# hengdashi/cuda_gcn

Measured on AMD Instinct MI355X. Metric: epochs_per_sec, higher is better.
Workload: dtype f32

## Files before the change

cuda_gcn_amd/_lib.py:

```python
from __future__ import annotations

import ctypes as C
import os

HERE = os.path.dirname(os.path.abspath(__file__))
LIBDIR = os.environ.get("GCN_LIBDIR") or os.path.join(HERE, "lib")

_cache = {}


class NativeLibraryMissing(RuntimeError):
    pass


def _load(name: str) -> C.CDLL:
    if name in _cache:
        return _cache[name]
    path = os.path.join(LIBDIR, name)
    if not os.path.exists(path):
        raise NativeLibraryMissing(
            f"{path} not found: the HIP extension is not built. Run `make kernels host` "
            f"(or __graft_entry__.build()); there is no CPU fallback.")
    try:
        lib = C.CDLL(path)
    except OSError as e:
        raise NativeLibraryMissing(f"cannot load {path}: {e}") from e
    _cache[name] = lib
    return lib


def gcnhip() -> C.CDLL:
    lib = _load("libgcnhip.so")
    if not getattr(lib, "_typed", False):
        _declare_gcnhip(lib)
        lib._typed = True
    return lib


def gcnhost() -> C.CDLL:
    gcnhip()
    lib = _load("libgcnhost.so")
    if not getattr(lib, "_typed", False):
        _declare_gcnhost(lib)
        lib._typed = True
    return lib


P = C.c_void_p
I = C.c_int
I64 = C.c_int64
U64 = C.c_uint64
F = C.c_float


class AdamVar(C.Structure):
    _fields_ = [("w", P), ("g", P), ("m", P), ("v", P), ("n", I64), ("decay", I)]


GCNHIP_SYMBOLS = {
    "gcnhip_device_count": (I, [C.POINTER(I)]),
    "gcnhip_ctx_create": (I, [C.POINTER(P), I, P]),
    "gcnhip_ctx_destroy": (I, [P]),
    "gcnhip_ctx_sync": (I, [P]),
    "gcnhip_ctx_set_corun": (I, [P, I]),
    "gcnhip_ctx_set_option": (I, [P, C.c_char_p, I]),
    "gcnhip_ctx_get_option": (I, [P, C.c_char_p, C.POINTER(I)]),
    "gcnhip_ctx_stream": (P, [P]),
    "gcnhip_error_string": (C.c_char_p, [I]),
    "gcnhip_last_error": (C.c_char_p, []),
    "gcnhip_version": (C.c_char_p, []),
    "gcnhip_experiments": (I, []),
    "gcnhip_malloc": (I, [P, C.POINTER(P), C.c_size_t]),
    "gcnhip_free": (I, [P, P]),
    "gcnhip_memset_async": (I, [P, P, I, C.c_size_t]),
    "gcnhip_h2d": (I, [P, P, P, C.c_size_t]),
    "gcnhip_d2h": (I, [P, P, P, C.c_size_t]),
    "gcnhip_d2d_async": (I, [P, P, P, C.c_size_t]),
    "gcnhip_host_alloc": (I, [C.POINTER(P), C.c_size_t]),
    "gcnhip_host_free": (I, [P]),
    "gcnhip_d2h_async": (I, [P, P, P, C.c_size_t]),
    "gcnhip_graph_create": (I, [P, C.POINTER(P), P, P, I, I, P]),
    "gcnhip_graph_create_grouped": (I, [P, C.POINTER(P), P, P, I, I, P, P]),
    "gcnhip_graph_set_schedule": (I, [P, P, I, P, I]),
    "gcnhip_graph_reserve_width": (I, [P, P, I]),
    "gcnhip_graph_destroy": (I, [P, P]),
    "gcnhip_graph_arrays": (I, [P, C.POINTER(P), C.POINTER(P), C.POINTER(P), C.POINTER(I), C.POINTER(I)]),
    "gcnhip_graphsum": (I, [P, P, P, I, P, I, I]),
    "gcnhip_graphsum_rowmask": (I, [P, P, P, I, P, I, I, P]),
    "gcnhip_graphsum_masked": (I, [P, P, P, I, P, I, I, P, P]),
    "gcnhip_graph_add_rowset": (I, [P, P, P, C.POINTER(P)]),
    "gcnhip_graph_create_restricted": (I, [P, C.POINTER(P), P, P]),
    "gcnhip_graph_clone": (I, [P, C.POINTER(P), P]),
    "gcnhip_rowset_size": (I, [P, C.POINTER(I)]),
    "gcnhip_graphsum_rowset": (I, [P, P, P, P, I, P, I, I, P]),
    "gcnhip_graphsum_relu_dropout": (I, [P, P, P, I, P, I, I, I, F, U64, P, U64, P]),
    "gcnhip_graphsum_relu_dropout_bits": (I, [P, P, P, I, P, I, I, I, F, U64, P, U64, P, P, I]),
    "gcnhip_graphsum_ex": (I, [P, P, P, P, I, P, I, I]),
    "gcnhip_graphsum_predict": (I, [P, P, P, P, P, I, P, I, I, I, P, P, P, I]),
    "gcnhip_graphsum_blend": (I, [P, P, P, I, P, I, P, I, I, F, F, F, F, P]),
    "gcnhip_cs_error_rows": (I, [P, P, I, P, I, P, I, I, P, I, P]),
    "gcnhip_cs_correct_rows": (I, [P, P, I, P, I, P, I, I, P, P, I]),
    "gcnhip_calib_nll_rows": (I, [P, P, I, P, I, P, I, I, F, P]),
    "gcnhip_calib_bins_rows": (I, [P, P, I, P, I, P, I, I, F, I, P, P, P]),
    "gcnhip_calib_scale_rows": (I, [P, P, I, I, P, I, I, F, P, I, P]),
    "gcnhip_embed_inv_norms": (I, [P, P, I, I, I, P]),
    "gcnhip_topk_plan": (I, [I, I, I, I, C.POINTER(I), C.POINTER(I), C.POINTER(C.c_size_t), C.POINTER(C.c_size_t)]),
    "gcnhip_topk_rows": (I, [P, P, I, I, I, P, P, P, I, I, I, I, P, C.c_size_t, I, P, P]),
    "gcnhip_pair_scores": (I, [P, P, I, I, I, P, P, P, I, P]),
    "gcnhip_embed_rows": (I, [P, P, I, I, I, P, P, I, P, I]),
    "gcnhip_graph_remove_rowset": (I, [P, P, P]),
    "gcnhip_graph_scales": (I, [P, C.POINTER(P), C.POINTER(P), C.POINTER(P), C.POINTER(P)]),
    "gcnhip_feat_scale_rows": (I, [P, P, P]),
    "gcnhip_xent_fwd_rows_scaled": (I, [P, P, I, P, I, P, P, I, I, I, I, I, P, P, P]),
    "gcnhip_xent_from_row_terms": (I, [P, P, P, P, I, P, P]),
    "gcnhip_matmul_bwd_ex": (I, [P, P, I, P, I, P, I, P, I, P, I, I, I, I, F, P, I, P]),
    "gcnhip_graphsum_part": (I, [P, P, P, P, I, P, I, I, P, I, I, I, F, U64, P, U64, P]),
    "gcnhip_feat_create": (I, [P, C.POINTER(P), P, P, P, I, I]),
    "gcnhip_feat_create_aggregated": (I, [P, C.POINTER(P), P, P]),
    "gcnhip_feat_destroy": (I, [P, P]),
    "gcnhip_feat_is_dense": (I, [P]),
    "gcnhip_feat_values": (P, [P]),
    "gcnhip_feat_nnz": (I64, [P]),
    "gcnhip_spmm_fwd": (I, [P, P, P, P, I, P, I, I, F, U64, P, U64, P]),
    "gcnhip_spmm_fwd_relu": (I, [P, P, P, P, I, P, I, I]),
    "gcnhip_spmm_fwd_relu_matmul": (I, [P, P, P, P, I, I, P, I, I, P, I]),
    "gcnhip_spmm_bwd": (I, [P, P, P, P, I, P, I, I, F, U64, P, U64, P]),
    "gcnhip_spmm_bwd_plan": (I, [P, P, I, C.POINTER(I), C.POINTER(I)]),
    "gcnhip_spmm_bwd_part": (I, [P, P, P, P, I, I, F, U64, P, U64, P, I, I, I]),
    "gcnhip_spmm_bwd_finish": (I, [P, P, P, I, I]),
    "gcnhip_matmul_fwd": (I, [P, P, I, P, I, P, I, I, I, I]),
    "gcnhip_matmul_bwd": (I, [P, P, I, P, I, P, I, P, I, P, I, I, I, I]),
    "gcnhip_matmul_bwd_fused": (I, [P, P, I, P, I, P, I, P, I, P, I, I, I, I, F]),
    "gcnhip_matmul_bwd_fused_bits": (I, [P, P, I, P, I, P, I, P, I, P, I, I, I, I, F, P, I]),
    "gcnhip_pack_positive": (I, [P, P, I, I, I, P, I]),
    "gcnhip_f32_to_bf16": (I, [P, P, I, P, I, I64, I]),
    "gcnhip_graphsum_bf16": (I, [P, P, P, I, P, I, I, P, P, I, I, F, U64, P, U64, P]),
    "gcnhip_matmul_bwd_da_bits": (I, [P, P, I, P, I, P, I, I, I, I, P, I, F]),
    "gcnhip_gather_rows": (I, [P, P, I, P, I, P]),
    "gcnhip_relu_fwd": (I, [P, P, P, I64, I]),
    "gcnhip_relu_bwd": (I, [P, P, P, I64]),
    "gcnhip_dropout_fwd": (I, [P, P, P, I64, F, U64, P, U64, P]),
    "gcnhip_dropout_bwd": (I, [P, P, P, I64, F]),
    "gcnhip_relu_fwd_2d": (I, [P, P, I, I, I, P, I]),
    "gcnhip_relu_bwd_2d": (I, [P, P, I, I, I, P]),
    "gcnhip_dropout_fwd_2d": (I, [P, P, I, I, I, P, F, U64, P, U64, P]),
    "gcnhip_dropout_bwd_2d": (I, [P, P, I, I, I, P, F]),
    "gcnhip_relu_dropout_bwd": (I, [P, P, I, P, I, I, I, F]),
    "gcnhip_xent_fwd": (I, [P, P, I, P, I, P, I, I, I, I, I, P, P]),
    "gcnhip_xent_fwd_rows": (I, [P, P, I, P, I, P, P, I, I, I, I, I, P, P]),
    "gcnhip_accuracy": (I, [P, P, I, P, I, I, P]),
    "gcnhip_set_truth": (I, [P, P, P, P, I, I]),
    "gcnhip_sumsq": (I, [P, P, I64, P]),
    "gcnhip_adam_step": (I, [P, C.POINTER(AdamVar), I, F, P, P, F, F, F, F, P]),
    "gcnhip_adam_step_advance": (I, [P, C.POINTER(AdamVar), I, F, P, P, F, F, F, F, P, P, P]),
    "gcnhip_counter_add": (I, [P, P, C.c_uint32]),
    "gcnhip_metrics_record": (I, [P, P, I, I, P, P, P, P]),
    "gcnhip_metrics_record_with_next_loss": (I, [P, P, I, I, P, P]),
    "gcnhip_capture_begin": (I, [P]),
    "gcnhip_capture_end": (I, [P, C.POINTER(P)]),
    "gcnhip_graph_launch": (I, [P, P]),
    "gcnhip_graph_exec_destroy": (I, [P]),
    "gcnhip_event_create": (I, [C.POINTER(P)]),
    "gcnhip_event_create_sync": (I, [C.POINTER(P)]),
    "gcnhip_event_destroy": (I, [P]),
    "gcnhip_event_record": (I, [P, P]),
    "gcnhip_stream_wait_event": (I, [P, P]),
    "gcnhip_event_elapsed_ms": (I, [P, P, C.POINTER(F)]),
    "gcnhip_event_sync": (I, [P]),
    "gcnhip_bce_fwd_rows": (I, [P, P, I, P, I, P, I, P, I, I, I, I, P, P, P]),
    "gcnhip_bce_predict_rows": (I, [P, P, I, P, I, I, P, I, P, I]),
    "gcnhip_confusion_rows": (I, [P, P, P, I, P, I, I, P, P]),
    "gcnhip_bce_class_counts_rows": (I, [P, P, I, P, I, P, I, I, P]),
    "gcnhip_wxent_fwd_rows": (I, [P, P, I, P, I, P, P, I, I, I, I, I, P, P, P, P, F]),
    "gcnhip_wbce_fwd_rows": (I, [P, P, I, P, I, P, I, P, I, I, I, I, P, P, P, P]),
}


def _declare_gcnhip(lib):
    for name, (res, args) in GCNHIP_SYMBOLS.items():
        fn = getattr(lib, name)
# ... 93 lines not shown
```

cuda_gcn_amd/csrc/dense_bf16x3.h:

```cpp
#pragma once
#include "dense_persist.h"
#include "bf16x3_split.h"

constexpr int BX_BK = 32;
constexpr int BX_BH_BYTES = 3 * 4 * 1024;
constexpr int BX_NB = 10;
constexpr int BX_PD = 6;
constexpr int BX_SMEM = BX_NB * BX_BH_BYTES;


__device__ inline void bx_pack_w_body(int idx, const float *__restrict__ w, int ldw, int K, int n_hs, uint4 *__restrict__ wp, float scale) {
    if (idx >= n_hs * 4 * 64) return;
    const int lane = idx & 63, n = (idx >> 6) & 3, hs = idx >> 8;
    const int col = 32 * n + (lane & 31), k0 = 32 * (hs >> 1) + 16 * (lane >> 5) + 8 * (hs & 1);
    BxPlanes P;
#pragma unroll
    for (int i = 0; i < 4; i++) {
        const int k = k0 + 2 * i;
        const float a = k < K ? w[(size_t)k * ldw + col] * scale : 0.f, b = (k + 1) < K ? w[(size_t)(k + 1) * ldw + col] * scale : 0.f;
        bx_split2(a, b, P.w[0][i], P.w[1][i], P.w[2][i]);
    }
#pragma unroll
    for (int p = 0; p < 3; p++) wp[(((size_t)hs * 3 + p) * 4 + n) * 64 + lane] = make_uint4(P.w[p][0], P.w[p][1], P.w[p][2], P.w[p][3]);
}
// ... 81 lines not shown
__global__ __launch_bounds__(256) void dropbits_bx_pack_w_kernel(BxBitsArgs b, int n_bits_wgs,
                                                                 const float *__restrict__ w, int ldw, int K, int n_hs,
                                                                 uint4 *__restrict__ wp, float scale) {
    __shared__ uint32_t lds[BX_BITS_LDS_WORDS];
    if ((int)blockIdx.x < n_bits_wgs) dropbits_cm_body(blockIdx.x, threadIdx.x, b, lds);
    else bx_pack_w_body(((int)blockIdx.x - n_bits_wgs) * 256 + threadIdx.x, w, ldw, K, n_hs, wp, scale);
}

struct Bx3FwdArgs {
    const float *x; int ldx;
    const uint4 *wp;
    float *out; int ldo;
    int m, K, n_chunks, n_rb;
    const uint32_t *bits;
    int relu;
    const uint4 *w2p;
    float *z0; int ldz, p2;
};
constexpr int BX_W2_BYTES = 8 * 2 * 3 * 1024;

struct BxB3 { bf16x8 h, m, l; };
template <int N> struct BxN { static constexpr int value = N; };
struct BxRaw { f32x4 v[4]; uint32_t kw; };

template <int OFF>
__device__ __forceinline__ void bx_gload16(f32x4 &dst, const float *p) {
    asm volatile("global_load_dwordx4 %0, %1, off offset:%2" : "=v"(dst) : "v"(p), "n"(OFF) : "memory");
}
__device__ __forceinline__ void bx_gload4(uint32_t &dst, const uint32_t *p) {
    asm volatile("global_load_dword %0, %1, off" : "=v"(dst) : "v"(p) : "memory");
}
template <int OFF>
__device__ __forceinline__ void bx_ldsread16(bf16x8 &dst, uint32_t addr) {
    asm volatile("ds_read_b128 %0, %1 offset:%2" : "=v"(dst) : "v"(addr), "n"(OFF) : "memory");
}
#define BX_WAIT_LDS(b) asm volatile("s_waitcnt lgkmcnt(0)" : "+v"((b).h), "+v"((b).m), "+v"((b).l) :: "memory")
#define BX_PIN(P, i) asm volatile("" : "+v"((P).w[0][i]), "+v"((P).w[1][i]), "+v"((P).w[2][i]))
#define BX_WAIT_RAW(N, r) asm volatile("s_waitcnt vmcnt(" #N ")" : "+v"((r).v[0]), "+v"((r).v[1]), "+v"((r).v[2]), "+v"((r).v[3]), "+v"((r).kw) :: "memory")

template <bool DROP, int NP, bool ZOUT = false>
__global__ __launch_bounds__(512, 2) void dense_fwd_bf16x3_kernel(Bx3FwdArgs a) {
    constexpr int NBV = ZOUT ? 8 : BX_NB;
    static_assert(NBV >= BX_PD + 1, "ring too short for the prefetch distance");
    __shared__ __attribute__((aligned(1024))) unsigned char smem[NBV * BX_BH_BYTES + (ZOUT ? BX_W2_BYTES : 0)];
    const int tid = threadIdx.x, lane = tid & 63;
    const int wave = __builtin_amdgcn_readfirstlane(tid >> 6);
    const int li = lane & 31, hh = lane >> 5;
    const uint32_t lds0 = (uint32_t)(uintptr_t)(__attribute__((address_space(3))) unsigned char *)smem;
    if (a.m < 0) smem[tid] = 0;

    const int rb_lo = (int)((int64_t)blockIdx.x * a.n_rb / gridDim.x);
    const int nb = (int)((int64_t)(blockIdx.x + 1) * a.n_rb / gridDim.x) - rb_lo;
    if (nb <= 0) return;
    const int row_last = min(a.m, (rb_lo + nb) * 32) - 1;
    const int n_rounds = (nb + 7) / 8;
    const int n_items = n_rounds * a.n_chunks;
    const int n_hs = 2 * a.n_chunks;
    const int piece2 = wave < 4 ? wave + 8 : wave - 4;

    auto load_raw = [&](BxRaw &r, int t, int c) __attribute__((always_inline)) {
        const int row = min((rb_lo + 8 * t + wave) * 32 + li, row_last);
        const float *p = a.x + (size_t)row * a.ldx + c * BX_BK + 16 * hh;
        if (DROP) bx_gload4(r.kw, a.bits + (size_t)c * a.m + row);
        bx_gload16<0>(r.v[0], p); bx_gload16<16>(r.v[1], p); bx_gload16<32>(r.v[2], p); bx_gload16<48>(r.v[3], p);
        if (!DROP) r.kw = 0u;
    };
    auto issue_b = [&](int hq) __attribute__((always_inline)) {
        int hs = hq % n_hs;
        const uint32_t dst = lds0 + (hq % NBV) * BX_BH_BYTES;
        const uint4 *src = a.wp + (size_t)hs * (BX_BH_BYTES / 16);
        pg_glds16(src + wave * 64 + lane, dst + wave * 1024);
        pg_glds16(src + piece2 * 64 + lane, dst + piece2 * 1024);
    };
    static_assert(2 * (BX_PD - 2) == 8, "BX_WAIT_W spells the count out");
#define BX_WAIT_W() PG_WAIT_BARRIER(8)

    f32x16 acc[4];
#pragma unroll
    for (int n = 0; n < 4; n++)
#pragma unroll
        for (int r = 0; r < 16; r++) acc[n][r] = 0.f;

    const __amdgpu_buffer_rsrc_t orsrc = __builtin_amdgcn_make_buffer_rsrc(a.out, 0, (int)((uint32_t)a.m * (uint32_t)a.ldo * 4u), 0x00020000);
    auto store_block = [&](f32x16 &v, int row0, int col, bool live) __attribute__((always_inline)) {
#pragma unroll
        for (int r = 0; r < 16; r++) {
            const int row = row0 + (r & 3) + 8 * (r >> 2) + 4 * hh;
            const float x = (a.relu && !(v[r] > 0.f)) ? 0.f : v[r];
            const uint32_t off = live ? ((uint32_t)row * (uint32_t)a.ldo + (uint32_t)col) * 4u : 0xFFFFFFF0u;
            __builtin_amdgcn_raw_buffer_store_b32(__float_as_uint(x), orsrc, (int)off, 0, 0);
            v[r] = 0.f;
        }
    };

    auto split_pair = [&](BxPlanes &P, const BxRaw &r, uint32_t win, int s, int i) __attribute__((always_inline)) {
        const f32x4 v = r.v[2 * s + (i >> 1)];
        float x0 = (i & 1) ? v[2] : v[0], x1 = (i & 1) ? v[3] : v[1];
        if (DROP) {
            const int j = 8 * s + 2 * i;
            x0 = __uint_as_float(__float_as_uint(x0) & (uint32_t)(((int32_t)(win << (31 - j))) >> 31));
            x1 = __uint_as_float(__float_as_uint(x1) & (uint32_t)(((int32_t)(win << (30 - j))) >> 31));
        }
        bx_split2(x0, x1, P.w[0][i], P.w[1][i], P.w[2][i]);
    };
    auto window = [&](const BxRaw &r, int t, int c) __attribute__((always_inline)) -> uint32_t {
        if (!DROP) return 0u;
        return r.kw >> (16 * hh);
    };
    auto read_b = [&](BxB3 &b, int hq, auto n_tag) __attribute__((always_inline)) {
        constexpr int N = decltype(n_tag)::value;
        const uint32_t addr = lds0 + (hq % NBV) * BX_BH_BYTES + lane * 16;
        bx_ldsread16<(0 * 4 + N) * 1024>(b.h, addr);
        bx_ldsread16<(1 * 4 + N) * 1024>(b.m, addr);
        bx_ldsread16<(2 * 4 + N) * 1024>(b.l, addr);
    };
    auto mac = [&](f32x16 &c, const BxPlanes &A, const BxB3 &B) __attribute__((always_inline)) {
        const bf16x8 ah = bx_plane(A, 0), am = bx_plane(A, 1), al = bx_plane(A, 2);
        if (ZOUT) {
            c = MFMA_BF16(B.h, al, c);
            c = MFMA_BF16(B.m, am, c);
            c = MFMA_BF16(B.l, ah, c);
            c = MFMA_BF16(B.h, am, c);
            c = MFMA_BF16(B.m, ah, c);
            c = MFMA_BF16(B.h, ah, c);
            return;
        }
        if (NP >= 8) { c = MFMA_BF16(al, B.m, c); c = MFMA_BF16(am, B.l, c); }
        c = MFMA_BF16(al, B.h, c);
        c = MFMA_BF16(am, B.m, c);
        c = MFMA_BF16(ah, B.l, c);
        c = MFMA_BF16(am, B.h, c);
        c = MFMA_BF16(ah, B.m, c);
        c = MFMA_BF16(ah, B.h, c);
    };
    auto second_product = [&](int row0, bool live) __attribute__((always_inline)) {
        const uint4 *img = reinterpret_cast<const uint4 *>(smem + NBV * BX_BH_BYTES);
        f32x16 z[2];
#pragma unroll
        for (int cb = 0; cb < 2; cb++)
#pragma unroll
            for (int r = 0; r < 16; r++) z[cb][r] = 0.f;
#pragma unroll
        for (int s = 0; s < 8; s++) {
            BxPlanes P;
#pragma unroll
            for (int i = 0; i < 4; i++) {
                float x0 = acc[s >> 1][8 * (s & 1) + 2 * i], x1 = acc[s >> 1][8 * (s & 1) + 2 * i + 1];
                x0 = (a.relu && !(x0 > 0.f)) ? 0.f : x0;
                x1 = (a.relu && !(x1 > 0.f)) ? 0.f : x1;
                bx_split2(x0, x1, P.w[0][i], P.w[1][i], P.w[2][i]);
            }
            const bf16x8 hh_ = bx_plane(P, 0), hm = bx_plane(P, 1), hl = bx_plane(P, 2);
#pragma unroll
            for (int cb = 0; cb < 2; cb++) {
                if (cb == 1 && a.p2 <= 32) continue;
                const int piece = s * 2 + cb;
                const bf16x8 wh = __builtin_bit_cast(bf16x8, img[(piece * 3 + 0) * 64 + lane]);
                const bf16x8 wm = __builtin_bit_cast(bf16x8, img[(piece * 3 + 1) * 64 + lane]);
                const bf16x8 wl = __builtin_bit_cast(bf16x8, img[(piece * 3 + 2) * 64 + lane]);
                z[cb] = MFMA_BF16(wl, hh_, z[cb]);
                z[cb] = MFMA_BF16(wm, hm, z[cb]);
                z[cb] = MFMA_BF16(wh, hl, z[cb]);
                z[cb] = MFMA_BF16(wm, hh_, z[cb]);
                z[cb] = MFMA_BF16(wh, hm, z[cb]);
                z[cb] = MFMA_BF16(wh, hh_, z[cb]);
            }
        }
#pragma unroll
        for (int n = 0; n < 4; n++)
#pragma unroll
            for (int r = 0; r < 16; r++) acc[n][r] = 0.f;
        const int row = row0 + li;
        if (live && row < a.m) {
            float *zp = a.z0 + (size_t)row * a.ldz;
#pragma unroll
            for (int cb = 0; cb < 2; cb++)
#pragma unroll
                for (int q = 0; q < 4; q++) {
                    const int c0 = 32 * cb + 8 * q + 4 * hh;
                    if (c0 + 4 <= a.p2) {
                        *reinterpret_cast<float4 *>(zp + c0) = make_float4(z[cb][4 * q], z[cb][4 * q + 1], z[cb][4 * q + 2], z[cb][4 * q + 3]);
                    } else {
#pragma unroll
                        for (int i = 0; i < 4; i++) if (c0 + i < a.p2) zp[c0 + i] = z[cb][4 * q + i];
                    }
                }
        }
    };
    auto interleave = [&]() __attribute__((always_inline)) {
#pragma unroll
        for (int k = 0; k < NP; k++) {
            __builtin_amdgcn_sched_group_barrier(0x008, 1, 0);
            __builtin_amdgcn_sched_group_barrier(0x002, 3, 0);
        }
    };

    if (ZOUT) {
        uint4 *img = reinterpret_cast<uint4 *>(smem + NBV * BX_BH_BYTES);
        for (int i = tid; i < BX_W2_BYTES / 16; i += 512) img[i] = a.w2p[i];
        __syncthreads();
    }
    BxRaw R0, R1, R2;
#pragma unroll
    for (int q = 0; q < BX_PD; q++) issue_b(q);
    load_raw(R0, 0, 0);
    {
        const int t1 = a.n_chunks > 1 ? 0 : 1, c1 = a.n_chunks > 1 ? 1 : 0;
        load_raw(R1, min(t1, n_rounds - 1), n_items > 1 ? c1 : 0);
    }
    BX_WAIT_RAW(0, R0);
    BX_WAIT_RAW(0, R1);
    __builtin_amdgcn_s_barrier();
    BxPlanes P0, P1;
    {
        const uint32_t w0 = window(R0, 0, 0);
#pragma unroll
        for (int i = 0; i < 4; i++) split_pair(P0, R0, w0, 0, i);
    }
    BxB3 Bc, Bn;
    read_b(Bc, 0, BxN<0>());
    BX_WAIT_LDS(Bc);

    auto chunk = [&](BxRaw &Ra, BxRaw &Rb, BxRaw &Rc, int g) __attribute__((always_inline)) {
        const int t = g / a.n_chunks, c = g - t * a.n_chunks;
        int t1 = t, c1 = c + 1; if (c1 == a.n_chunks) { c1 = 0; ++t1; }
        int t2 = t1, c2 = c1 + 1; if (c2 == a.n_chunks) { c2 = 0; ++t2; }
        if (t1 >= n_rounds) { t1 = n_rounds - 1; c1 = a.n_chunks - 1; }
        if (t2 >= n_rounds) { t2 = n_rounds - 1; c2 = a.n_chunks - 1; }
        const int h0 = 2 * g;
        const uint32_t wa = window(Ra, t, c);
        read_b(Bn, h0, BxN<1>());
        __builtin_amdgcn_sched_barrier(0);
        split_pair(P1, Ra, wa, 1, 0);
        mac(acc[0], P0, Bc);
        interleave();
        BX_PIN(P1, 0);
        __builtin_amdgcn_sched_barrier(0);
        BX_WAIT_LDS(Bn);
        read_b(Bc, h0, BxN<2>());
        __builtin_amdgcn_sched_barrier(0);
        split_pair(P1, Ra, wa, 1, 1);
        mac(acc[1], P0, Bn);
        interleave();
        BX_PIN(P1, 1);
        __builtin_amdgcn_sched_barrier(0);
        BX_WAIT_LDS(Bc);
        BX_WAIT_W();
        issue_b(h0 + BX_PD);
        load_raw(Rc, t2, c2);
        read_b(Bn, h0, BxN<3>());
        __builtin_amdgcn_sched_barrier(0);
        split_pair(P1, Ra, wa, 1, 2);
        mac(acc[2], P0, Bc);
        interleave();
        BX_PIN(P1, 2);
        __builtin_amdgcn_sched_barrier(0);
        BX_WAIT_LDS(Bn);
        read_b(Bc, h0 + 1, BxN<0>());
        __builtin_amdgcn_sched_barrier(0);
        split_pair(P1, Ra, wa, 1, 3);
        mac(acc[3], P0, Bn);
        interleave();
        BX_PIN(P1, 3);
        __builtin_amdgcn_sched_barrier(0);
        BX_WAIT_LDS(Bc);
        if (DROP) BX_WAIT_RAW(5, Rb); else BX_WAIT_RAW(4, Rb);
        const uint32_t wb = window(Rb, t1, c1);
        read_b(Bn, h0 + 1, BxN<1>());
        __builtin_amdgcn_sched_barrier(0);
        split_pair(P0, Rb, wb, 0, 0);
        mac(acc[0], P1, Bc);
        interleave();
        BX_PIN(P0, 0);
        __builtin_amdgcn_sched_barrier(0);
        BX_WAIT_LDS(Bn);
        read_b(Bc, h0 + 1, BxN<2>());
        __builtin_amdgcn_sched_barrier(0);
        split_pair(P0, Rb, wb, 0, 1);
        mac(acc[1], P1, Bn);
        interleave();
        BX_PIN(P0, 1);
        __builtin_amdgcn_sched_barrier(0);
        BX_WAIT_LDS(Bc);
        BX_WAIT_W();
        issue_b(h0 + 1 + BX_PD);
        read_b(Bn, h0 + 1, BxN<3>());
        __builtin_amdgcn_sched_barrier(0);
        split_pair(P0, Rb, wb, 0, 2);
        mac(acc[2], P1, Bc);
        interleave();
        BX_PIN(P0, 2);
        __builtin_amdgcn_sched_barrier(0);
        BX_WAIT_LDS(Bn);
        read_b(Bc, h0 + 2, BxN<0>());
        __builtin_amdgcn_sched_barrier(0);
        split_pair(P0, Rb, wb, 0, 3);
        mac(acc[3], P1, Bn);
        interleave();
        BX_PIN(P0, 3);
        __builtin_amdgcn_sched_barrier(0);
        BX_WAIT_LDS(Bc);
        if (c == a.n_chunks - 1) {
            const bool live = 8 * t + wave < nb;
            if (ZOUT) {
                second_product((rb_lo + 8 * t + wave) * 32, live);
            } else {
#pragma unroll
                for (int n = 0; n < 4; n++) store_block(acc[n], (rb_lo + 8 * t + wave) * 32, 32 * n + li, live);
            }
        }
    };
    int g = 0;
    for (; g + 3 <= n_items; g += 3) {
        chunk(R0, R1, R2, g);
        chunk(R1, R2, R0, g + 1);
        chunk(R2, R0, R1, g + 2);
    }
    if (g < n_items) {
        chunk(R0, R1, R2, g); g++;
        if (g < n_items) { chunk(R1, R2, R0, g); g++; }
    }
    BX_WAIT_RAW(0, R0);
    BX_WAIT_RAW(0, R1);
    BX_WAIT_RAW(0, R2);
}
#undef BX_WAIT_W


struct Bx3BwdArgs {
    const float *x; int ldx;
    const float *dout; int ldd;
    float *slab; int p_ld;
    int m, K, rps;
    int split0;
    const uint32_t *bits;
    float scale;
};

template <int OFF>
__device__ __forceinline__ void bx_ldswrite16(uint32_t addr, u32x4 v) {
    asm volatile("ds_write_b128 %0, %1 offset:%2" :: "v"(addr), "v"(v), "n"(OFF) : "memory");
}
__device__ __forceinline__ float bx_keep(float x, uint64_t lane_mask) {
    float y;
    asm("v_cndmask_b32_e64 %0, 0, %1, %2" : "=v"(y) : "v"(x), "s"(lane_mask));
    return y;
}
struct BxRaw8 { float a[8], b[8]; uint32_t k; };
#define BX_WAIT_RAW8(N, r) asm volatile("s_waitcnt vmcnt(" #N ")" : "+v"((r).a[0]), "+v"((r).a[1]), "+v"((r).a[2]), "+v"((r).a[3]), "+v"((r).a[4]), "+v"((r).a[5]), "+v"((r).a[6]), "+v"((r).a[7]), \
                                                                   "+v"((r).b[0]), "+v"((r).b[1]), "+v"((r).b[2]), "+v"((r).b[3]), "+v"((r).b[4]), "+v"((r).b[5]), "+v"((r).b[6]), "+v"((r).b[7]), \
                                                                   "+v"((r).k) :: "memory")

template <bool DROP, int NP>
__global__ __launch_bounds__(256, 2) void dense_bwd_bf16x3_kernel(Bx3BwdArgs a) {
    __shared__ __attribute__((aligned(1024))) unsigned char smem[2 * BX_BH_BYTES];
    const int tid = threadIdx.x, lane = tid & 63;
    const int wave = __builtin_amdgcn_readfirstlane(tid >> 6);
    const int li = lane & 31, hh = lane >> 5;
    const uint32_t lds0 = (uint32_t)(uintptr_t)(__attribute__((address_space(3))) unsigned char *)smem;
    if (a.m < 0) smem[tid] = 0;
    const int fr = blockIdx.x, split = blockIdx.y + a.split0;
    const int F0 = 128 * fr + 32 * wave;
    const int r_lo = split * a.rps, r_hi = min(a.m, r_lo + a.rps);
    const int n_steps = r_hi > r_lo ? (r_hi - r_lo + 15) >> 4 : 0;

    const u32x4 rs_x = bx_make_rsrc(a.x, (uint32_t)a.m * (uint32_t)a.ldx * 4u);
    const u32x4 rs_d = bx_make_rsrc(a.dout, (uint32_t)a.m * (uint32_t)a.ldd * 4u);
    uint32_t so_x[8], so_d[8];
#pragma unroll
    for (int j = 0; j < 8; j++) { so_x[j] = (uint32_t)j * (uint32_t)a.ldx * 4u; so_d[j] = (uint32_t)j * (uint32_t)a.ldd * 4u; }
    const uint32_t vo_x0 = ((uint32_t)(r_lo + 8 * hh) * (uint32_t)a.ldx + (uint32_t)(F0 + li)) * 4u;
    const uint32_t vo_d0 = ((uint32_t)(r_lo + 8 * hh) * (uint32_t)a.ldd + (uint32_t)(32 * wave + li)) * 4u;
    const uint32_t step_x = 16u * (uint32_t)a.ldx * 4u, step_d = 16u * (uint32_t)a.ldd * 4u;
    const u32x4 rs_k = bx_make_rsrc(a.bits, (uint32_t)((a.K + 31) / 32) * (uint32_t)a.m * 4u);
    const uint32_t vo_k0 = ((uint32_t)(F0 >> 5) * (uint32_t)a.m + (uint32_t)(r_lo + (lane & 15))) * 4u;
    auto load_raw = [&](BxRaw8 &r, int s) __attribute__((always_inline)) {
        const uint32_t vx = vo_x0 + (uint32_t)s * step_x, vd = vo_d0 + (uint32_t)s * step_d;
        if (DROP) {
            asm volatile("buffer_load_dword %0, %1, %2, 0 offen" : "=v"(r.k) : "v"(vo_k0 + (uint32_t)s * 64u), "s"(rs_k) : "memory");
#pragma unroll
            for (int j = 0; j < 8; j++) { bx_bload4(r.a[j], vx, rs_x, so_x[j]); bx_bload4(r.b[j], vd, rs_d, so_d[j]); }
        } else {
#pragma unroll
            for (int j = 0; j < 8; j++) bx_bload4(r.a[j], vx, rs_x, so_x[j]);
#pragma unroll
            for (int j = 0; j < 8; j++) bx_bload4(r.b[j], vd, rs_d, so_d[j]);
            r.k = 0u;
        }
    };
    struct Masks { uint64_t m[8]; };
    auto field = [&](int row) __attribute__((always_inline)) -> uint32_t {
        return row < r_hi ? 0xFFFFFFFFu : 0u;
    };
    auto make_masks = [&](Masks &M, int s, const BxRaw8 &r) __attribute__((always_inline)) {
        const int r0 = r_lo + 16 * s;
#pragma unroll
        for (int j = 0; j < 8; j++) {
            uint32_t lo = field(r0 + j), hi = field(r0 + 8 + j);
            if (DROP) {
                lo &= (uint32_t)__builtin_amdgcn_readlane((int)r.k, j);
                hi &= (uint32_t)__builtin_amdgcn_readlane((int)r.k, 8 + j);
            }
            M.m[j] = (uint64_t)lo | ((uint64_t)hi << 32);
            asm volatile("" : "+s"(M.m[j]));
        }
    };
    auto split_a_pair = [&](BxPlanes &P, const BxRaw8 &r, const Masks &M, int s, int i) __attribute__((always_inline)) {
        const float x0 = bx_keep(r.a[2 * i], M.m[2 * i]), x1 = bx_keep(r.a[2 * i + 1], M.m[2 * i + 1]);
        bx_split2(x0, x1, P.w[0][i], P.w[1][i], P.w[2][i]);
    };
    auto split_b_pair = [&](BxPlanes &P, const BxRaw8 &r, int i) __attribute__((always_inline)) {
        bx_split2(r.b[2 * i], r.b[2 * i + 1], P.w[0][i], P.w[1][i], P.w[2][i]);
    };
    auto write_b = [&](const BxPlanes &P, int slot) __attribute__((always_inline)) {
        const uint32_t addr = lds0 + slot * BX_BH_BYTES + (wave * 64 + lane) * 16;
        bx_ldswrite16<0 * 4096>(addr, (u32x4){P.w[0][0], P.w[0][1], P.w[0][2], P.w[0][3]});
        bx_ldswrite16<1 * 4096>(addr, (u32x4){P.w[1][0], P.w[1][1], P.w[1][2], P.w[1][3]});
        bx_ldswrite16<2 * 4096>(addr, (u32x4){P.w[2][0], P.w[2][1], P.w[2][2], P.w[2][3]});
    };
    auto read_b = [&](BxB3 &b, int slot, auto n_tag) __attribute__((always_inline)) {
        constexpr int N = decltype(n_tag)::value;
        const uint32_t addr = lds0 + slot * BX_BH_BYTES + lane * 16;
        bx_ldsread16<(0 * 4 + N) * 1024>(b.h, addr);
        bx_ldsread16<(1 * 4 + N) * 1024>(b.m, addr);
        bx_ldsread16<(2 * 4 + N) * 1024>(b.l, addr);
    };
    auto mac = [&](f32x16 &c, const BxPlanes &A, const BxB3 &B) __attribute__((always_inline)) {
        const bf16x8 ah = bx_plane(A, 0), am = bx_plane(A, 1), al = bx_plane(A, 2);
        if (NP >= 8) { c = MFMA_BF16(al, B.m, c); c = MFMA_BF16(am, B.l, c); }
        c = MFMA_BF16(al, B.h, c);
        c = MFMA_BF16(am, B.m, c);
        c = MFMA_BF16(ah, B.l, c);
        c = MFMA_BF16(am, B.h, c);
        c = MFMA_BF16(ah, B.m, c);
        c = MFMA_BF16(ah, B.h, c);
    };
    auto interleave = [&]() __attribute__((always_inline)) {
#pragma unroll
        for (int k = 0; k < NP; k++) {
            __builtin_amdgcn_sched_group_barrier(0x008, 1, 0);
            __builtin_amdgcn_sched_group_barrier(0x002, 4, 0);
        }
    };

    f32x16 acc[4];
#pragma unroll
    for (int n = 0; n < 4; n++)
#pragma unroll
        for (int r = 0; r < 16; r++) acc[n][r] = 0.f;

    if (n_steps > 0) {
        BxRaw8 R0, R1;
        load_raw(R0, 0);
        load_raw(R1, 1);
        if (DROP) BX_WAIT_RAW8(17, R0); else BX_WAIT_RAW8(16, R0);
        BxPlanes PA0, PA1, PB;
        Masks M;
        make_masks(M, 0, R0);
#pragma unroll
        for (int i = 0; i < 4; i++) { split_a_pair(PA0, R0, M, 0, i); split_b_pair(PB, R0, i); }
        write_b(PB, 0);
        asm volatile("s_waitcnt lgkmcnt(0)\n\ts_barrier" ::: "memory");
        BxB3 Bc, Bn;
        read_b(Bc, 0, BxN<0>());
        BX_WAIT_LDS(Bc);
        auto step = [&](BxPlanes &PAc, BxPlanes &PAn, BxRaw8 &Rn, BxRaw8 &Rf, int s) __attribute__((always_inline)) {
            const int slot = s & 1;
            load_raw(Rf, s + 2);
            if (DROP) BX_WAIT_RAW8(17, Rn); else BX_WAIT_RAW8(16, Rn);
            make_masks(M, s + 1, Rn);
            read_b(Bn, slot, BxN<1>());
            __builtin_amdgcn_sched_barrier(0);
            split_b_pair(PB, Rn, 0); split_b_pair(PB, Rn, 1);
            mac(acc[0], PAc, Bc);
            interleave();
            BX_PIN(PB, 0); BX_PIN(PB, 1);
            __builtin_amdgcn_sched_barrier(0);
            BX_WAIT_LDS(Bn);
            read_b(Bc, slot, BxN<2>());
            __builtin_amdgcn_sched_barrier(0);
            split_b_pair(PB, Rn, 2); split_b_pair(PB, Rn, 3);
            mac(acc[1], PAc, Bn);
            interleave();
            BX_PIN(PB, 2); BX_PIN(PB, 3);
            __builtin_amdgcn_sched_barrier(0);
            BX_WAIT_LDS(Bc);
            write_b(PB, slot ^ 1);
            read_b(Bn, slot, BxN<3>());
            __builtin_amdgcn_sched_barrier(0);
            split_a_pair(PAn, Rn, M, s + 1, 0); split_a_pair(PAn, Rn, M, s + 1, 1);
            mac(acc[2], PAc, Bc);
            interleave();
            BX_PIN(PAn, 0); BX_PIN(PAn, 1);
            __builtin_amdgcn_sched_barrier(0);
            BX_WAIT_LDS(Bn);
            split_a_pair(PAn, Rn, M, s + 1, 2); split_a_pair(PAn, Rn, M, s + 1, 3);
            mac(acc[3], PAc, Bn);
            interleave();
            BX_PIN(PAn, 2); BX_PIN(PAn, 3);
            __builtin_amdgcn_sched_barrier(0);
            asm volatile("s_waitcnt lgkmcnt(0)\n\ts_barrier" ::: "memory");
            read_b(Bc, slot ^ 1, BxN<0>());
            BX_WAIT_LDS(Bc);
        };
        int s = 0;
        for (; s + 2 <= n_steps; s += 2) {
            step(PA0, PA1, R1, R0, s);
            step(PA1, PA0, R0, R1, s + 1);
        }
        if (s < n_steps) step(PA0, PA1, R1, R0, s);
        BX_WAIT_RAW8(0, R0);
        BX_WAIT_RAW8(0, R1);
    }
    float *slab = a.slab + (size_t)split * a.K * a.p_ld;
#pragma unroll
    for (int n = 0; n < 4; n++)
#pragma unroll
        for (int r = 0; r < 16; r++) {
            const int feat = F0 + (r & 3) + 8 * (r >> 2) + 4 * hh;
            if (feat < a.K) slab[(size_t)feat * a.p_ld + 32 * n + li] = acc[n][r] * a.scale;
        }
}
```

cuda_gcn_amd/csrc/graphsum.hip:

```cpp
#include "dense_kernels.h"
#include <algorithm>
#include <stdlib.h>

struct GsArgs {
    const int *indptr, *indices;
    const float *coef;
    const int4 *tasks;
    int n_tasks, n_rows, nnz;
    size_t table_bytes;
    const float *in;
    const uint16_t *in_bf;
    float *out;
    float *partials;
    int ld_in, ld_out, part_ld, dim;
    int n_slices;
    int bounds[9];
    int fuse, training, thr;
    float scale;
    uint64_t seed, elem_offset;
    const uint32_t *d_epoch;
    const uint8_t *keep_mask;
    const uint32_t *row_bits;
    const uint32_t *out_bits;
    uint32_t *pos_bits;
    int wpr;
    int accumulate;
    const float *post;
    const int32_t *xe_truth;
    float *xe_grad; int xe_ld_grad; int xe_training;
    float xe_count;
    const float *xe_grad_scale;
    float *xe_terms;
};

__device__ inline bool row_wanted(const GsArgs &a, int row) {
    return !a.out_bits || ((a.out_bits[row >> 5] >> (row & 31)) & 1u);
}

__device__ inline float4 f4_fma(float c, float4 v, float4 a) {
    a.x += c * v.x; a.y += c * v.y; a.z += c * v.z; a.w += c * v.w;
    return a;
}
__device__ inline float4 f4_add(float4 a, float4 b) { return make_float4(a.x + b.x, a.y + b.y, a.z + b.z, a.w + b.w); }
__device__ inline float4 f4_shfl_xor(float4 v, int m) {
    return make_float4(__shfl_xor(v.x, m, WAVE), __shfl_xor(v.y, m, WAVE), __shfl_xor(v.z, m, WAVE), __shfl_xor(v.w, m, WAVE));
}

__device__ inline float4 relu_dropout4(float4 v, const GsArgs &a, int64_t r, int col0) {
    float x[4] = {v.x, v.y, v.z, v.w};
#pragma unroll
    for (int i = 0; i < 4; i++) x[i] = x[i] > 0.f ? x[i] : 0.f;
    if (a.training) {
        const uint32_t epoch = a.d_epoch ? *a.d_epoch : 0u;
        const int64_t e0 = r * a.dim + col0;
        uint32_t bits;
        if (a.keep_mask) {
            bits = 0;
#pragma unroll
            for (int i = 0; i < 4; i++) bits |= (col0 + i < a.dim && a.keep_mask[e0 + i] ? 1u : 0u) << i;
        } else {
            const uint64_t j0 = a.elem_offset + (uint64_t)e0;
            if ((j0 & 3) == 0) {
                bits = keep4(j0 >> 2, epoch, a.seed, a.thr);
            } else {
                bits = 0;
#pragma unroll
                for (int i = 0; i < 4; i++) bits |= (keep1(j0 + i, epoch, a.seed, a.thr) ? 1u : 0u) << i;
            }
        }
#pragma unroll
        for (int i = 0; i < 4; i++) x[i] *= (bits >> i & 1u) ? a.scale : 0.f;
    }
    return make_float4(x[0], x[1], x[2], x[3]);
}

template <int L>
__device__ __forceinline__ void xent_row_epilogue4(const GsArgs &a, int row, float4 z, int lane, int l, int g, int col0) {
#pragma clang fp contract(off)
    const int t = a.xe_truth[row];
    const int nv4 = (a.dim + 3) >> 2;
    float *gr = a.xe_grad ? a.xe_grad + (size_t)row * a.xe_ld_grad : nullptr;
    if (t < 0) {
        if (a.xe_training && gr && g == 0 && l < nv4) *reinterpret_cast<float4 *>(gr + col0) = make_float4(0.f, 0.f, 0.f, 0.f);
        if (lane == 0) *reinterpret_cast<float2 *>(a.xe_terms + 2 * (size_t)row) = make_float2(0.f, 0.f);
        return;
    }
    float x[4] = {z.x, z.y, z.z, z.w};
    float mx = -1e30f;
#pragma unroll
    for (int i = 0; i < 4; i++) if (col0 + i < a.dim) mx = fmaxf(mx, x[i]);
#pragma unroll
    for (int m = 1; m < L; m <<= 1) mx = fmaxf(mx, __shfl_xor(mx, m, WAVE));
    mx = __int_as_float(__builtin_amdgcn_readfirstlane(__float_as_int(mx)));
    const int ti = t & 3;
    const float sel = ti == 0 ? x[0] : (ti == 1 ? x[1] : (ti == 2 ? x[2] : x[3]));
    const float tv = __int_as_float(__builtin_amdgcn_readlane(__float_as_int(sel), t >> 2));
    const bool correct = !(mx > tv);
    float ex[4];
#pragma unroll
    for (int i = 0; i < 4; i++) {
        x[i] -= mx;
        ex[i] = col0 + i < a.dim ? expf(x[i]) : 0.f;
    }
    float se = 0.f;
    for (int q = 0; q < nv4; q++) {
#pragma unroll
        for (int i = 0; i < 4; i++) se += __int_as_float(__builtin_amdgcn_readlane(__float_as_int(ex[i]), q));
    }
    const float term = logf(se) - (tv - mx);
    if (lane == 0) *reinterpret_cast<float2 *>(a.xe_terms + 2 * (size_t)row) = make_float2(term, correct ? 1.f : 0.f);
    if (a.xe_training && gr && g == 0 && l < nv4) {
        const float gs = a.xe_grad_scale ? a.xe_grad_scale[row] : 1.f;
        float o[4];
#pragma unroll
        for (int i = 0; i < 4; i++) {
            float p = ex[i] / se;
            if (col0 + i == t) p = (float)((double)p - 1.0);
            o[i] = col0 + i < a.dim ? (a.xe_grad_scale ? (p / a.xe_count) * gs : p / a.xe_count) : 0.f;
        }
        *reinterpret_cast<float4 *>(gr + col0) = make_float4(o[0], o[1], o[2], o[3]);
    }
}
__device__ __forceinline__ void xent_row_epilogue1(const GsArgs &a, int row, float v, int lane) {
#pragma clang fp contract(off)
    const int t = a.xe_truth[row];
    const int nv4 = (a.dim + 3) >> 2;
    float *gr = a.xe_grad ? a.xe_grad + (size_t)row * a.xe_ld_grad : nullptr;
    if (t < 0) {
        if (a.xe_training && gr && lane < 4 * nv4) gr[lane] = 0.f;
        if (lane == 0) *reinterpret_cast<float2 *>(a.xe_terms + 2 * (size_t)row) = make_float2(0.f, 0.f);
        return;
    }
    float mx = lane < a.dim ? fmaxf(-1e30f, v) : -1e30f;
#pragma unroll
    for (int m = 1; m < WAVE; m <<= 1) mx = fmaxf(mx, __shfl_xor(mx, m, WAVE));
    const float tv = __int_as_float(__builtin_amdgcn_readlane(__float_as_int(v), t));
    const bool correct = !(mx > tv);
    const float x = v - mx;
    const float ex = lane < a.dim ? expf(x) : 0.f;
    float se = 0.f;
    for (int j = 0; j < 4 * nv4; j++) se += __int_as_float(__builtin_amdgcn_readlane(__float_as_int(ex), j));
    const float term = logf(se) - (tv - mx);
    if (lane == 0) *reinterpret_cast<float2 *>(a.xe_terms + 2 * (size_t)row) = make_float2(term, correct ? 1.f : 0.f);
    if (a.xe_training && gr && lane < 4 * nv4) {
        float p = ex / se;
// ... 451 lines not shown
        v.x = (h[0] & 0xFFFFu) | (h[1] << 16); v.y = (h[2] & 0xFFFFu) | (h[3] << 16);
        v.z = (h[4] & 0xFFFFu) | (h[5] << 16); v.w = (h[6] & 0xFFFFu) | (h[7] << 16);
        *reinterpret_cast<uint4 *>(dst + r * ld_dst + c0) = v;
    }
}

template <int L>
static void launch_bf16(GsArgs a, const int (*xb)[9], hipStream_t s, const PredArgs *pred = nullptr) {
    const int ychunks = ceil_div(a.dim, L * 8);
    const bool sliced = ychunks > 1 && 8 % ychunks == 0;
    a.n_slices = sliced ? ychunks : 1;
    const int G = 8 / a.n_slices;
    const int lg = G == 8 ? 3 : (G == 4 ? 2 : (G == 2 ? 1 : 0));
    int max_blocks = 1;
    for (int k = 0; k <= 8; k++) a.bounds[k] = xb[lg][k];
    for (int k = 0; k < G; k++) max_blocks = std::max(max_blocks, ceil_div(a.bounds[k + 1] - a.bounds[k], 4));
    if constexpr (L <= 8) {
        if (pred) { graphsum_predict_bf16_kernel<L><<<max_blocks * 8, 256, 0, s>>>(a, *pred); return; }
    }
    graphsum_bf16_kernel<L><<<dim3(max_blocks * 8, sliced ? 1 : ychunks), 256, 0, s>>>(a);
}

template <int L>
__global__ __launch_bounds__(256) void graphsum_scalar_kernel(GsArgs a) {
    constexpr int G = WAVE / L;
    constexpr int MAXC = 4;
    const int lane = threadIdx.x & 63;
    const int t = blockIdx.x * (blockDim.x >> 6) + (threadIdx.x >> 6);
    const int nt = a.n_tasks ? a.n_tasks : a.n_rows;
    if (t >= nt) return;
    int row, e0, e1, slot;
    if (a.n_tasks) {
        const int4 tk = a.tasks[t];
        row = tk.x; e0 = tk.y; e1 = tk.z; slot = tk.w;
    } else {
        row = t; e0 = a.indptr[t]; e1 = a.indptr[t + 1]; slot = -1;
    }
    if (!row_wanted(a, row)) return;
    const int g = lane / L, l = lane % L;
    for (int cbase = 0; cbase < a.dim; cbase += L * MAXC) {
        float acc[MAXC] = {0.f, 0.f, 0.f, 0.f};
        for (int base = e0; base < e1; base += WAVE) {
            const int cnt = min(WAVE, e1 - base);
            int my_idx = 0;
            float my_c = 0.f;
            if (lane < cnt) {
                my_idx = a.indices[base + lane];
                my_c = a.coef[base + lane];
                if (a.row_bits && !((a.row_bits[my_idx >> 5] >> (my_idx & 31)) & 1u)) my_c = 0.f;
            }
            const int iters = (cnt + G - 1) / G;
#pragma unroll 4
            for (int k = 0; k < iters; k++) {
                const int src = k * G + g;
                const int j = __shfl(my_idx, src, WAVE);
                const float c = __shfl(my_c, src, WAVE);
                const float *p = a.in + (size_t)j * a.ld_in + cbase + l;
                if (src < cnt && c != 0.f) {
#pragma unroll
                    for (int q = 0; q < MAXC; q++)
                        if (cbase + l + q * L < a.dim) acc[q] += c * p[q * L];
                }
            }
        }
#pragma unroll
        for (int q = 0; q < MAXC; q++) {
#pragma unroll
            for (int m = L; m < WAVE; m <<= 1) acc[q] += __shfl_xor(acc[q], m, WAVE);
        }
        if (g == 0) {
#pragma unroll
            for (int q = 0; q < MAXC; q++) {
                const int col = cbase + l + q * L;
                if (col >= a.dim) continue;
                float v = acc[q];
                if (slot >= 0) {
                    a.partials[(size_t)slot * a.part_ld + col] = v;
                } else {
                    if (a.accumulate) v = a.out[(size_t)row * a.ld_out + col] + v;
                    if (a.fuse) {
                        v = v > 0.f ? v : 0.f;
                        if (a.training) {
                            const int64_t e = (int64_t)row * a.dim + col;
                            const bool keep = a.keep_mask ? a.keep_mask[e] != 0
                                                          : keep1(a.elem_offset + (uint64_t)e, a.d_epoch ? *a.d_epoch : 0u, a.seed, a.thr);
                            v *= keep ? a.scale : 0.f;
                        }
                    }
                    a.out[(size_t)row * a.ld_out + col] = v;
                }
            }
        }
    }
}

__global__ __launch_bounds__(256) void graphsum_finalize_kernel(GsArgs a, const int4 *split_rows, int n_split_rows) {
    const int s = blockIdx.x;
    if (s >= n_split_rows) return;
    const int4 sr = split_rows[s];
    const int row = sr.x, first = sr.y, ns = sr.z;
    if (!row_wanted(a, row)) return;
    for (int c0 = 0; c0 < a.dim; c0 += blockDim.x) {
        const int col = c0 + threadIdx.x;
        float v = 0.f;
        if (col < a.dim) {
            v = a.accumulate ? a.out[(size_t)row * a.ld_out + col] : 0.f;
            const float *pp = a.partials + (size_t)first * a.part_ld + col;
            int k = 0;
            for (; k + 4 <= ns; k += 4) {
                const float p0 = pp[(size_t)k * a.part_ld], p1 = pp[(size_t)(k + 1) * a.part_ld];
                const float p2 = pp[(size_t)(k + 2) * a.part_ld], p3 = pp[(size_t)(k + 3) * a.part_ld];
                v += p0; v += p1; v += p2; v += p3;
            }
            {
                const float p0 = pp[(size_t)min(k, ns - 1) * a.part_ld], p1 = pp[(size_t)min(k + 1, ns - 1) * a.part_ld];
                const float p2 = pp[(size_t)min(k + 2, ns - 1) * a.part_ld];
                if (k < ns) v += p0;
                if (k + 1 < ns) v += p1;
                if (k + 2 < ns) v += p2;
            }
            if (a.post) v *= a.post[row];
            if (a.fuse) {
                v = v > 0.f ? v : 0.f;
                if (a.training) {
                    const int64_t e = (int64_t)row * a.dim + col;
                    const bool keep = a.keep_mask ? a.keep_mask[e] != 0
                                                  : keep1(a.elem_offset + (uint64_t)e, a.d_epoch ? *a.d_epoch : 0u, a.seed, a.thr);
                    v *= keep ? a.scale : 0.f;
                }
            }
            a.out[(size_t)row * a.ld_out + col] = v;
        }
        if (a.xe_truth && threadIdx.x < WAVE) xent_row_epilogue1(a, row, v, threadIdx.x);
        if (a.pos_bits) {
            const uint64_t b = __ballot(col < a.dim && v > 0.f);
            const int w0 = (c0 + (int)(threadIdx.x & ~63u)) >> 5;
            if ((threadIdx.x & 63) == 0 && w0 < a.wpr) a.pos_bits[(size_t)row * a.wpr + w0] = (uint32_t)b;
            if ((threadIdx.x & 63) == 32 && w0 + 1 < a.wpr) a.pos_bits[(size_t)row * a.wpr + w0 + 1] = (uint32_t)(b >> 32);
        }
    }
}

__global__ __launch_bounds__(256) void graphsum_finalize_predict_kernel(GsArgs a, PredArgs p, const int4 *split_rows, int n_split_rows) {
    const int s = blockIdx.x;
    if (s >= n_split_rows || threadIdx.x >= WAVE) return;
    const int4 sr = split_rows[s];
    const int row = sr.x, first = sr.y, ns = sr.z;
    const int col = threadIdx.x;
    float v = 0.f;
    if (col < a.dim) {
        const float *pp = a.partials + (size_t)first * a.part_ld + col;
        int k = 0;
        for (; k + 4 <= ns; k += 4) {
            const float p0 = pp[(size_t)k * a.part_ld], p1 = pp[(size_t)(k + 1) * a.part_ld];
            const float p2 = pp[(size_t)(k + 2) * a.part_ld], p3 = pp[(size_t)(k + 3) * a.part_ld];
            v += p0; v += p1; v += p2; v += p3;
        }
        for (; k < ns; k++) v += pp[(size_t)k * a.part_ld];
        if (a.post) v *= a.post[row];
        if (a.out) a.out[(size_t)row * a.ld_out + col] = v;
    }
    predict_row_epilogue1(a, p, row, v, col);
}

struct BlendArgs {
    const float *base;
    int ld_base;
    float alpha, beta, lo, hi;
    int32_t *pred;
};

__device__ __forceinline__ float blend1(const BlendArgs &b, float sum, float base) {
#pragma clang fp contract(off)
    return fminf(fmaxf(b.alpha * sum + b.beta * base, b.lo), b.hi);
}

template <int L, int U>
__global__ __launch_bounds__(256) void graphsum_blend_vec_kernel(GsArgs a, BlendArgs b) {
    const int lane = threadIdx.x & 63;
    int t;
    {
        const int xcd = blockIdx.x & 7, q = blockIdx.x >> 3;
        t = a.bounds[xcd] + q * (blockDim.x >> 6) + (threadIdx.x >> 6);
        if (t >= a.bounds[xcd + 1]) return;
    }
    int row, e0, e1, slot;
    if (a.n_tasks) {
        const int4 tk = a.tasks[t];
        row = tk.x; e0 = tk.y; e1 = tk.z; slot = tk.w;
    } else {
        row = t; e0 = a.indptr[t]; e1 = a.indptr[t + 1]; slot = -1;
    }
    const int g = lane / L, l = lane % L;
    const int col0 = l * 4;
    const bool active = col0 < a.dim;
    const float *in = a.in + (active ? col0 : 0);
    float4 acc = make_float4(0.f, 0.f, 0.f, 0.f);
    for (int base = e0; base < e1; base += WAVE) {
        const int cnt = min(WAVE, e1 - base);
        int my_idx = 0;
        float my_c = 0.f;
        if (lane < cnt) {
            my_idx = a.indices[base + lane];
            my_c = a.coef[base + lane];
        }
        acc = gather_chunk<L, U>(a, in, my_idx, my_c, cnt, g, acc);
    }
#pragma unroll
    for (int m = L; m < WAVE; m <<= 1) acc = f4_add(acc, f4_shfl_xor(acc, m));
    if (slot >= 0) {
// ... 20 lines not shown
    if (b.pred) {
#pragma unroll
        for (int m = 1; m < L; m <<= 1) argmax_merge(bv, bi, __shfl_xor(bv, m, WAVE), __shfl_xor(bi, m, WAVE));
        if (lane == 0) b.pred[row] = bi;
    }
}

__global__ __launch_bounds__(64) void graphsum_finalize_blend_kernel(GsArgs a, BlendArgs b, const int4 *split_rows, int n_split_rows) {
    const int s = blockIdx.x;
    if (s >= n_split_rows || threadIdx.x >= WAVE) return;
    const int4 sr = split_rows[s];
    const int row = sr.x, first = sr.y, ns = sr.z;
    const int col = threadIdx.x;
    const bool in_row = col < a.dim;
    float v = 0.f;
    if (in_row) {
        const float *pp = a.partials + (size_t)first * a.part_ld + col;
        int k = 0;
        for (; k + 4 <= ns; k += 4) {
            const float p0 = pp[(size_t)k * a.part_ld], p1 = pp[(size_t)(k + 1) * a.part_ld];
            const float p2 = pp[(size_t)(k + 2) * a.part_ld], p3 = pp[(size_t)(k + 3) * a.part_ld];
            v += p0; v += p1; v += p2; v += p3;
        }
        for (; k < ns; k++) v += pp[(size_t)k * a.part_ld];
        v = blend1(b, v, b.base[(size_t)row * b.ld_base + col]);
        a.out[(size_t)row * a.ld_out + col] = v;
    }
    if (b.pred) {
        float bv = in_row ? v : -INFINITY;
        int bi = in_row ? col : 0x7FFFFFFF;
#pragma unroll
        for (int m = 1; m < WAVE; m <<= 1) argmax_merge(bv, bi, __shfl_xor(bv, m, WAVE), __shfl_xor(bi, m, WAVE));
        if (col == 0) b.pred[row] = bi;
    }
}

template <int L>
static void launch_blend(const GsArgs &a, const BlendArgs &b, int blocks, int u, hipStream_t s) {
    if (u >= 4) graphsum_blend_vec_kernel<L, 4><<<blocks, 256, 0, s>>>(a, b);
    else graphsum_blend_vec_kernel<L, 2><<<blocks, 256, 0, s>>>(a, b);
}

template <int L>
static void launch_vec(GsArgs &a, const int (*xb)[9], const gcnhip_ctx *c, const PredArgs *pred = nullptr) {
    hipStream_t s = c->stream;
    const int ychunks = ceil_div(a.dim, L * 4);
    const bool sliced = ychunks > 1 && 8 % ychunks == 0;
    a.n_slices = sliced ? ychunks : 1;
    const int G = 8 / a.n_slices;
    const int lg = G == 8 ? 3 : (G == 4 ? 2 : (G == 2 ? 1 : 0));
    int max_blocks = 1;
    for (int k = 0; k <= 8; k++) a.bounds[k] = xb[lg][k];
    for (int k = 0; k < G; k++) max_blocks = std::max(max_blocks, ceil_div(a.bounds[k + 1] - a.bounds[k], 4));
    const int force_u = c->opt.gs_u;
    const int u = force_u ? force_u : (a.table_bytes > ((size_t)256 << 20) ? 2 : 4);
    const dim3 grid(max_blocks * 8, sliced ? 1 : ychunks);
    if constexpr (L <= 16) {
        if (pred) {
            if (u >= 4) graphsum_predict_vec_kernel<L, 4><<<grid, 256, 0, s>>>(a, *pred);
            else graphsum_predict_vec_kernel<L, 2><<<grid, 256, 0, s>>>(a, *pred);
            return;
        }
    }
    if (sliced) {
        if (u >= 4) graphsum_vec_kernel<L, 4, true><<<grid, 256, 0, s>>>(a);
        else if (u >= 2) graphsum_vec_kernel<L, 2, true><<<grid, 256, 0, s>>>(a);
        else graphsum_vec_kernel<L, 1, true><<<grid, 256, 0, s>>>(a);
    } else {
        if (u >= 4) graphsum_vec_kernel<L, 4><<<grid, 256, 0, s>>>(a);
        else if (u >= 2) graphsum_vec_kernel<L, 2><<<grid, 256, 0, s>>>(a);
        else graphsum_vec_kernel<L, 1><<<grid, 256, 0, s>>>(a);
    }
}
template <int L>
static void launch_scalar(const GsArgs &a, int nt, hipStream_t s) {
    graphsum_scalar_kernel<L><<<ceil_div(nt, 4), 256, 0, s>>>(a);
}

static int graphsum_impl(gcnhip_ctx *c, const gcnhip_graph *g, const float *in, int ld_in, float *out, int ld_out,
                         int dim, int fuse, int training, float p, uint64_t seed, const uint32_t *d_epoch,
                         uint64_t elem_offset, const uint8_t *keep_mask, const uint32_t *row_bits = nullptr,
                         const uint16_t *in_bf = nullptr, const uint32_t *out_bits = nullptr,
                         const gcnhip_rowset *rs = nullptr, int accumulate = 0, uint32_t *pos_bits = nullptr, int wpr = 0, int scaling = 0,
                         const gcnhip_gs_loss *loss = nullptr, const PredArgs *pred = nullptr) {
    if (!c || !g || (!in && !in_bf) || (!out && !pred) || dim <= 0 || ld_in < dim || ld_out < dim) return -1;
    if (scaling < 0 || scaling > 3) return -1;
    if (accumulate && in_bf) return -1;
    if (rs && rs->owner != g)
        return gcnhip_fail("gcnhip_graphsum*: the row subset was registered on another adjacency object");
    if (in_bf && (ld_in % 8 != 0 || !aligned16(in_bf))) return -1;
    if (g->n_rows == 0 || (rs && rs->n_tasks == 0)) return 0;
    if (g->n_slots && g->part_ld < (dim + 7) / 8 * 8)
        return gcnhip_fail("gcnhip_graphsum*: dim is wider than the split-row scratch of this adjacency object; call "
                           "gcnhip_graph_reserve_width(ctx, g, dim) once before the first launch (restricted objects: on them too)");
    GsArgs a;
    a.indptr = g->indptr; a.indices = g->indices; a.coef = g->coef;
    a.tasks = rs ? rs->tasks : g->tasks; a.n_tasks = rs ? rs->n_tasks : g->n_tasks; a.n_rows = g->n_rows; a.nnz = g->nnz;
    a.table_bytes = (size_t)g->n_cols * ld_in * (in_bf ? 2 : 4);
    const int (*xb)[9] = rs ? rs->bounds : g->bounds;
    const int4 *split_rows = rs ? rs->split_rows : g->split_rows;
    const int n_split_rows = rs ? rs->n_split_rows : g->n_split_rows;
    a.in = in; a.in_bf = in_bf; a.out = out; a.partials = g->partials;
    a.ld_in = ld_in; a.ld_out = ld_out; a.part_ld = g->part_ld; a.dim = dim;
    a.fuse = fuse; a.training = training; a.thr = dropout_threshold(p);
    a.scale = 1 / (1 - p);
    a.seed = seed; a.elem_offset = elem_offset; a.d_epoch = d_epoch; a.keep_mask = keep_mask;
    a.row_bits = row_bits;
    a.out_bits = out_bits;
    a.accumulate = accumulate;
    a.pos_bits = pos_bits; a.wpr = wpr;
    a.post = nullptr;
    const int nt = a.n_tasks ? a.n_tasks : g->n_rows;
    const bool vec = (ld_in % 4 == 0) && (ld_out % 4 == 0) && aligned16(in) && aligned16(out);
    a.xe_truth = nullptr; a.xe_grad = nullptr; a.xe_ld_grad = 0; a.xe_training = 0; a.xe_count = 1.f; a.xe_grad_scale = nullptr; a.xe_terms = nullptr;
    if (loss) {
        const int w4 = (dim + 3) / 4 * 4;
        if (in_bf || !vec || dim > 64 || fuse || pos_bits || !loss->truth || !loss->row_terms || loss->count <= 0 || ((uintptr_t)loss->row_terms & 7))
            return gcnhip_fail("gcnhip_graphsum_ex: the loss epilogue needs f32 rows that are 16-byte aligned, dim <= 64, no relu_dropout, truth, row_terms and count > 0");
        if (loss->training && (!loss->grad || loss->ld_grad < w4 || loss->ld_grad % 4 != 0 || !aligned16(loss->grad)))
            return gcnhip_fail("gcnhip_graphsum_ex: the loss epilogue writes whole 16-byte quads of the gradient row: ld_grad % 4 == 0, ld_grad >= round_up(dim, 4)");
        a.xe_truth = loss->truth; a.xe_grad = loss->training ? loss->grad : nullptr; a.xe_ld_grad = loss->ld_grad; a.xe_training = loss->training ? 1 : 0;
        a.xe_count = (float)loss->count; a.xe_grad_scale = loss->grad_row_scale; a.xe_terms = loss->row_terms;
    }
    if (pred && (dim > 64 || fuse || pos_bits || loss || accumulate || row_bits || out_bits || (!in_bf && !vec)))
        return gcnhip_fail("gcnhip_graphsum_predict: needs dim <= 64 and f32 rows that are 16-byte aligned (ld % 4 == 0) or a bf16 table");
    if (scaling) {
        if (in_bf || !vec) return gcnhip_fail("gcnhip_graphsum_ex: scaling != 0 needs f32 rows that are 16-byte aligned (ld % 4 == 0)");
        a.coef = nullptr;
        a.post = scaling == 1 ? g->dinv_row : (scaling == 2 ? g->dinv2_row : nullptr);
    }
    if (pos_bits && !(fuse && !in_bf && vec && dim % 32 == 0 && wpr * 32 >= dim))
        return gcnhip_fail("gcnhip_graphsum_relu_dropout_bits: needs the fused epilogue, 16-byte aligned rows, dim % 32 == 0 and words_per_row * 32 >= dim");
    const int d4 = (dim + 3) / 4;
    a.n_slices = 1;
    if (in_bf) {
        const int d8 = (dim + 7) / 8;
        if (d8 <= 1) launch_bf16<1>(a, xb, c->stream, pred);
        else if (d8 <= 2) launch_bf16<2>(a, xb, c->stream, pred);
        else if (d8 <= 4) launch_bf16<4>(a, xb, c->stream, pred);
        else if (d8 % 16 == 0) launch_bf16<16>(a, xb, c->stream);
        else launch_bf16<8>(a, xb, c->stream, pred);
    }
    const int gl = c->opt.gs_l;
    if (in_bf) {
    } else if (vec && !loss && !pred && (gl == 8 || (gl == 4 && !pos_bits)) && dim % (gl * 4) == 0 && dim / (gl * 4) > 1 && 8 % (dim / (gl * 4)) == 0) {
        if (gl == 8) launch_vec<8>(a, xb, c); else launch_vec<4>(a, xb, c);
    } else if (vec && dim % 64 == 0 && 8 % (dim / 64) == 0) {
        launch_vec<16>(a, xb, c, pred);
    } else if (vec) {
        if (d4 <= 1) launch_vec<1>(a, xb, c, pred);
        else if (d4 <= 2) launch_vec<2>(a, xb, c, pred);
        else if (d4 <= 4) launch_vec<4>(a, xb, c, pred);
        else if (d4 <= 8) launch_vec<8>(a, xb, c, pred);
        else if (d4 <= 16) launch_vec<16>(a, xb, c, pred);
        else if (d4 <= 32) launch_vec<32>(a, xb, c);
        else launch_vec<64>(a, xb, c);
    } else {
        if (dim <= 1) launch_scalar<1>(a, nt, c->stream);
        else if (dim <= 2) launch_scalar<2>(a, nt, c->stream);
        else if (dim <= 4) launch_scalar<4>(a, nt, c->stream);
        else if (dim <= 8) launch_scalar<8>(a, nt, c->stream);
        else if (dim <= 16) launch_scalar<16>(a, nt, c->stream);
        else if (dim <= 32) launch_scalar<32>(a, nt, c->stream);
        else launch_scalar<64>(a, nt, c->stream);
    }
    GCNHIP_LAUNCH_CHECK();
    if (n_split_rows) {
        if (pred) graphsum_finalize_predict_kernel<<<n_split_rows, WAVE, 0, c->stream>>>(a, *pred, split_rows, n_split_rows);
        else graphsum_finalize_kernel<<<n_split_rows, 256, 0, c->stream>>>(a, split_rows, n_split_rows);
        GCNHIP_LAUNCH_CHECK();
    }
    return 0;
}

extern "C" {

int gcnhip_graphsum(gcnhip_ctx *c, const gcnhip_graph *g, const float *in, int ld_in,
                    float *out, int ld_out, int dim) {
    return graphsum_impl(c, g, in, ld_in, out, ld_out, dim, 0, 0, 0.f, 0, nullptr, 0, nullptr);
}

int gcnhip_graphsum_rowmask(gcnhip_ctx *c, const gcnhip_graph *g, const float *in, int ld_in,
                            float *out, int ld_out, int dim, const uint32_t *in_row_bits) {
    return graphsum_impl(c, g, in, ld_in, out, ld_out, dim, 0, 0, 0.f, 0, nullptr, 0, nullptr, in_row_bits);
}

int gcnhip_graphsum_masked(gcnhip_ctx *c, const gcnhip_graph *g, const float *in, int ld_in,
                           float *out, int ld_out, int dim, const uint32_t *in_row_bits, const uint32_t *out_row_bits) {
    return graphsum_impl(c, g, in, ld_in, out, ld_out, dim, 0, 0, 0.f, 0, nullptr, 0, nullptr, in_row_bits, nullptr, out_row_bits);
}

int gcnhip_graphsum_rowset(gcnhip_ctx *c, const gcnhip_graph *g, const gcnhip_rowset *rows, const float *in, int ld_in,
                           float *out, int ld_out, int dim, const uint32_t *in_row_bits) {
    if (!rows) return -1;
    return graphsum_impl(c, g, in, ld_in, out, ld_out, dim, 0, 0, 0.f, 0, nullptr, 0, nullptr, in_row_bits, nullptr, nullptr, rows);
}

int gcnhip_graphsum_relu_dropout(gcnhip_ctx *c, const gcnhip_graph *g, const float *in, int ld_in,
                                 float *out, int ld_out, int dim, int training, float p,
                                 uint64_t seed, const uint32_t *d_epoch, uint64_t elem_offset,
                                 const uint8_t *keep_mask) {
    if (training && !(p >= 0.f && p < 1.f)) return -1;
    return graphsum_impl(c, g, in, ld_in, out, ld_out, dim, 1, training, p, seed, d_epoch, elem_offset, keep_mask);
}

int gcnhip_graphsum_relu_dropout_bits(gcnhip_ctx *c, const gcnhip_graph *g, const float *in, int ld_in,
                                      float *out, int ld_out, int dim, int training, float p,
                                      uint64_t seed, const uint32_t *d_epoch, uint64_t elem_offset,
                                      const uint8_t *keep_mask, uint32_t *pos_bits, int words_per_row) {
    if (training && !(p >= 0.f && p < 1.f)) return -1;
    if (!pos_bits) return -1;
    return graphsum_impl(c, g, in, ld_in, out, ld_out, dim, 1, training, p, seed, d_epoch, elem_offset, keep_mask, nullptr, nullptr, nullptr,
                         nullptr, 0, pos_bits, words_per_row);
}

int gcnhip_graphsum_part(gcnhip_ctx *c, const gcnhip_graph *g, const gcnhip_rowset *rows, const float *in, int ld_in,
                         float *out, int ld_out, int dim, const uint32_t *in_row_bits, int accumulate,
                         int relu_dropout, int training, float p, uint64_t seed, const uint32_t *d_epoch,
                         uint64_t elem_offset, const uint8_t *keep_mask) {
    if (relu_dropout && training && !(p >= 0.f && p < 1.f)) return -1;
    return graphsum_impl(c, g, in, ld_in, out, ld_out, dim, relu_dropout ? 1 : 0, relu_dropout ? training : 0, relu_dropout ? p : 0.f,
                         seed, d_epoch, elem_offset, keep_mask, in_row_bits, nullptr, nullptr, rows, accumulate ? 1 : 0);
}

int gcnhip_graphsum_ex(gcnhip_ctx *c, const gcnhip_graph *g, const gcnhip_gs_opts *o, const float *in, int ld_in, float *out, int ld_out, int dim) {
    if (!o) return -1;
    if (o->relu_dropout && o->training && !(o->p >= 0.f && o->p < 1.f)) return -1;
    if (o->pos_bits && !o->relu_dropout) return -1;
    return graphsum_impl(c, g, in, ld_in, out, ld_out, dim, o->relu_dropout ? 1 : 0, o->relu_dropout ? o->training : 0, o->relu_dropout ? o->p : 0.f,
                         o->seed, o->d_epoch, o->elem_offset, o->keep_mask, o->in_row_bits, nullptr, nullptr, o->rows, o->accumulate ? 1 : 0,
                         o->pos_bits, o->words_per_row, o->scaling, o->loss);
}

int gcnhip_graphsum_predict(gcnhip_ctx *c, const gcnhip_graph *g, const gcnhip_rowset *rows, const float *in, const uint16_t *in_bf16,
                            int ld_in, float *out, int ld_out, int dim, int scaling, int32_t *pred, float *prob, float *logp, int ld_logp) {
    if (!pred || !prob || (in != nullptr) == (in_bf16 != nullptr)) return -1;
    if (logp && ld_logp < dim) return -1;
    if (in_bf16 && scaling) return gcnhip_fail("gcnhip_graphsum_predict: the factored operator (scaling != 0) gathers f32 rows only");
    const PredArgs pa = {pred, prob, logp, ld_logp};
    return graphsum_impl(c, g, in, ld_in, out, out ? ld_out : (dim + 3) / 4 * 4, dim, 0, 0, 0.f, 0, nullptr, 0, nullptr, nullptr, in_bf16, nullptr, rows, 0,
                         nullptr, 0, scaling, nullptr, &pa);
}

int gcnhip_graphsum_blend(gcnhip_ctx *c, const gcnhip_graph *g, const float *in, int ld_in, const float *base, int ld_base,
                          float *out, int ld_out, int dim, float alpha, float beta, float lo, float hi, int32_t *pred) {
    if (!c || !g || !in || !base || !out) return gcnhip_fail("gcnhip_graphsum_blend: null argument");
    if (dim < 1 || dim > 64) return gcnhip_fail("gcnhip_graphsum_blend: 1 <= dim <= 64 (the row of a node sits in one lane group)");
    if (ld_in < dim || ld_base < dim || ld_out < dim || ld_in % 4 || ld_base % 4 || ld_out % 4 || !aligned16(in) || !aligned16(base) || !aligned16(out))
        return gcnhip_fail("gcnhip_graphsum_blend: needs f32 rows that are 16-byte aligned (ld % 4 == 0, ld >= dim)");
    if (out == in) return gcnhip_fail("gcnhip_graphsum_blend: out must not be in (other rows are still gathering it); base may be");
    if (g->n_rows == 0) return 0;
    if (g->n_slots && g->part_ld < (dim + 7) / 8 * 8)
        return gcnhip_fail("gcnhip_graphsum_blend: dim is wider than the split-row scratch of this adjacency object; call gcnhip_graph_reserve_width");
    GsArgs a = {};
    a.indptr = g->indptr; a.indices = g->indices; a.coef = g->coef;
    a.tasks = g->tasks; a.n_tasks = g->n_tasks; a.n_rows = g->n_rows; a.nnz = g->nnz;
    a.table_bytes = (size_t)g->n_cols * ld_in * 4;
    a.in = in; a.out = out; a.partials = g->partials;
    a.ld_in = ld_in; a.ld_out = ld_out; a.part_ld = g->part_ld; a.dim = dim;
    a.n_slices = 1;
    int max_blocks = 1;
    for (int k = 0; k <= 8; k++) a.bounds[k] = g->bounds[3][k];
    for (int k = 0; k < 8; k++) max_blocks = std::max(max_blocks, ceil_div(a.bounds[k + 1] - a.bounds[k], 4));
    const BlendArgs b = {base, ld_base, alpha, beta, lo, hi, pred};
    const int u = c->opt.gs_u ? c->opt.gs_u : (a.table_bytes > ((size_t)256 << 20) ? 2 : 4);
    const int d4 = (dim + 3) / 4, blocks = max_blocks * 8;
    if (d4 <= 1) launch_blend<1>(a, b, blocks, u, c->stream);
    else if (d4 <= 2) launch_blend<2>(a, b, blocks, u, c->stream);
    else if (d4 <= 4) launch_blend<4>(a, b, blocks, u, c->stream);
    else if (d4 <= 8) launch_blend<8>(a, b, blocks, u, c->stream);
    else launch_blend<16>(a, b, blocks, u, c->stream);
    GCNHIP_LAUNCH_CHECK();
    if (g->n_split_rows) {
        graphsum_finalize_blend_kernel<<<g->n_split_rows, WAVE, 0, c->stream>>>(a, b, g->split_rows, g->n_split_rows);
        GCNHIP_LAUNCH_CHECK();
    }
    return 0;
}

int gcnhip_f32_to_bf16(gcnhip_ctx *c, const float *src, int ld_src, uint16_t *dst, int ld_dst, int64_t rows, int dim) {
    if (!c || !src || !dst || rows < 0 || dim <= 0 || ld_src < dim || ld_dst < dim || ld_dst % 8 != 0 || !aligned16(dst)) return -1;
    if (rows == 0) return 0;
    int64_t blocks = (rows * (ld_dst / 8) + 255) / 256;
    if (blocks > 65536) blocks = 65536;
    f32_to_bf16_kernel<<<(int)blocks, 256, 0, c->stream>>>(src, ld_src, dst, ld_dst, rows, dim);
    GCNHIP_LAUNCH_CHECK();
    return 0;
}

int gcnhip_graphsum_bf16(gcnhip_ctx *c, const gcnhip_graph *g, const uint16_t *in_bf16, int ld_in,
                         float *out, int ld_out, int dim, const uint32_t *in_row_bits, const gcnhip_rowset *out_rows,
                         int relu_dropout, int training, float p, uint64_t seed, const uint32_t *d_epoch,
                         uint64_t elem_offset, const uint8_t *keep_mask) {
    if (relu_dropout && training && !(p >= 0.f && p < 1.f)) return -1;
    return graphsum_impl(c, g, nullptr, ld_in, out, ld_out, dim, relu_dropout ? 1 : 0, training, relu_dropout ? p : 0.f, seed, d_epoch,
                         elem_offset, keep_mask, in_row_bits, in_bf16, nullptr, out_rows);
}

}

GCNHIP_DEFINE_PRELOAD(graphsum, graphsum_finalize_kernel)
```

cuda_gcn_amd/csrc/spmm.hip:

```cpp
#include "dense_kernels.h"
#include "dense_tile128.h"
#include "dense_persist.h"
#include "dense_bf16x3.h"
#include "spmm_sparse.h"
#include <limits.h>

struct DenseFwdArgs {
    const float *x; int ldx;
    const float *w; int ldw;
    float *out; int ldo;
    int m, K, p;
    const uint32_t *bits;
    float scale;
    int relu;
};

constexpr int DF_BM = 128, DF_BK = 32;
constexpr int DF_ALD = DF_BK + 2;

template <int NT, int VX>
__global__ __launch_bounds__(256) void spmm_dense_fwd_kernel(DenseFwdArgs a) {
    constexpr int BN = NT * 16;
    constexpr int BLD = BN + 16;
    __shared__ __attribute__((aligned(16))) float As[DF_BM * DF_ALD];
// ... 251 lines not shown
                         float *out, int ld_out, int p, float p_drop, uint64_t seed, const uint32_t *d_epoch,
                         uint64_t nnz_offset, const uint8_t *keep_mask, int relu, const Z0Fuse *zf = nullptr) {
    if (!c || !f || !vals || !w || (!out && !zf) || p <= 0 || ld_w < p || (out && ld_out < p)) return -1;
    if (!(p_drop >= 0.f && p_drop < 1.f)) return -1;
    if (zf && !(f->dense && p == 128)) return GCNHIP_NOT_AVAILABLE;
    if (f->n_rows == 0) return 0;
    const DropSpec d = make_drop(p_drop, seed, d_epoch, nnz_offset, keep_mask);
    if (f->dense && p > 64) {
        if (d.on && !f->keep_bits) return gcnhip_fail("input dropout on a feature object without a keep-bit array (gcnhip_feat_create_aggregated builds evaluation-only objects)");
        Tile128Args t;
        t.x = vals; t.ldx = f->n_cols; t.w = w; t.ldw = ld_w; t.out = out; t.ldo = ld_out;
        int vx = x_vec_width(f, vals);
        if (vals == f->values && f->values_pad) { t.x = f->values_pad; t.ldx = f->ld_pad; vx = 4; }
        t.m = f->n_rows; t.K = f->n_cols; t.p = p; t.bits = d.on ? f->keep_bits : nullptr; t.scale = d.scale; t.rows_per_split = 0; t.relu = relu;
        const bool fast = vx == 4 && t.ldx % 4 == 0 && (t.K + 31) / 32 * 32 <= t.ldx && ld_w % 4 == 0 && p % T_BN == 0 && aligned16(w);
        int rc = dense_fwd_bf16x3(c, f, t, d, fast, zf);
        if (rc == NOT_MINE) rc = dense_fwd_persist(c, f, t, d, fast);
        if (rc == NOT_MINE) rc = dense_fwd_tiles(c, f, t, d, fast, vx);
        return rc;
    }
    if (f->dense) {
        if (d.on) { const int rc = make_keep_bits(c, f, d); if (rc) return rc; }
        DenseFwdArgs a;
        a.x = vals; a.ldx = f->n_cols; a.w = w; a.ldw = ld_w; a.out = out; a.ldo = ld_out;
        a.m = f->n_rows; a.K = f->n_cols; a.p = p; a.bits = d.on ? f->keep_bits : nullptr; a.scale = d.scale; a.relu = relu;
        int vx = x_vec_width(f, vals);
        if (vals == f->values && f->values_pad) { a.x = f->values_pad; a.ldx = f->ld_pad; vx = 4; }
        const int nt_total = ceil_div(p, 16);
        const int NT = nt_total >= 8 ? 8 : (nt_total > 4 ? 8 : (nt_total > 2 ? 4 : nt_total));
        dim3 grid(ceil_div(f->n_rows, DF_BM), ceil_div(nt_total, NT));
        switch (NT) {
            case 1: launch_dense_fwd<1>(a, vx, grid, c->stream); break;
            case 2: launch_dense_fwd<2>(a, vx, grid, c->stream); break;
            case 4: launch_dense_fwd<4>(a, vx, grid, c->stream); break;
            default: launch_dense_fwd<8>(a, vx, grid, c->stream); break;
        }
        GCNHIP_LAUNCH_CHECK();
        return 0;
    }
    SpFwdArgs a;
    a.indptr = f->indptr; a.indices = f->indices; a.vals = vals; a.w = w; a.out = out;
    a.n_rows = f->n_rows; a.ld_w = ld_w; a.ld_out = ld_out; a.p = p; a.d = d; a.relu = relu;
    a.w_floats = f->n_cols * ld_w;
    a.rows_per_wave = 1;
    const bool vec = ld_w % 4 == 0 && aligned16(w);
    const int units = vec ? (p + 3) / 4 : p;
    a.nnz_bytes = (int)std::min<int64_t>(f->nnz * 4, 0x7FFFFFFF);
    a.rows_per_wave = std::max(1, std::min(8, (int)(f->n_rows / ((int64_t)c->n_cu * 64))));
    if (c->opt.spmm_rows > 0) a.rows_per_wave = std::min(32, c->opt.spmm_rows);
    a.n_slices = 1;
    if (vec && c->opt.spmm_slices != 0 && p % 32 == 0 && (p / 32 == 2 || p / 32 == 4 || p / 32 == 8) &&
        (size_t)f->n_cols * ld_w * sizeof(float) > ((size_t)4 << 20) && f->n_rows >= 8 * 64) {
        a.n_slices = p / 32;
        if (c->opt.spmm_rows <= 0) a.rows_per_wave = 2;
        const int Gs = 8 / a.n_slices;
        const int units_total = ceil_div(f->n_rows, a.rows_per_wave);
        const int per_group = ceil_div(units_total, Gs) + 1;
        dim3 sgrid(8 * ceil_div(per_group, 4), 1);
        a.nnz_bytes = (int)std::min<int64_t>(f->nnz * 4, 0x7FFFFFFF);
        spmm_csr_fwd_kernel<8, true, true><<<sgrid, 256, 0, c->stream>>>(a);
        GCNHIP_LAUNCH_CHECK();
        return 0;
    }
    dim3 grid(ceil_div(ceil_div(f->n_rows, a.rows_per_wave), 4), 1);
    a.nnz_bytes = (int)std::min<int64_t>(f->nnz * 4, 0x7FFFFFFF);
    const bool narrow = vec && units <= 16 && f->nnz * 4 < 0x7FFFFFFF && !c->opt.spmm_general && (f->nnz >= SPMM_NARROW_MIN_NNZ || c->opt.spmm_general < 0);
    if (narrow) {
        if (units <= 1) spmm_csr_fwd_q_kernel<1><<<grid, 256, 0, c->stream>>>(a);
        else if (units <= 2) spmm_csr_fwd_q_kernel<2><<<grid, 256, 0, c->stream>>>(a);
        else if (units <= 4) spmm_csr_fwd_q_kernel<4><<<grid, 256, 0, c->stream>>>(a);
        else if (units <= 8) spmm_csr_fwd_q_kernel<8><<<grid, 256, 0, c->stream>>>(a);
        else spmm_csr_fwd_q_kernel<16><<<grid, 256, 0, c->stream>>>(a);
        GCNHIP_LAUNCH_CHECK();
        return 0;
    }
#define SPF(L_)                                                                           \
    do {                                                                                  \
        if (vec) spmm_csr_fwd_kernel<L_, true><<<grid, 256, 0, c->stream>>>(a);           \
        else spmm_csr_fwd_kernel<L_, false><<<grid, 256, 0, c->stream>>>(a);              \
    } while (0)
    if (units <= 1) SPF(1); else if (units <= 2) SPF(2); else if (units <= 4) SPF(4);
    else if (units <= 8) SPF(8); else if (units <= 16) SPF(16); else if (units <= 32) SPF(32); else SPF(64);
#undef SPF
    GCNHIP_LAUNCH_CHECK();
    return 0;
}

int gcnhip_spmm_fwd(gcnhip_ctx *c, const gcnhip_feat *f, const float *vals, const float *w, int ld_w,
                    float *out, int ld_out, int p, float p_drop, uint64_t seed, const uint32_t *d_epoch,
                    uint64_t nnz_offset, const uint8_t *keep_mask) {
    return spmm_fwd_impl(c, f, vals, w, ld_w, out, ld_out, p, p_drop, seed, d_epoch, nnz_offset, keep_mask, 0);
}

int gcnhip_spmm_fwd_relu(gcnhip_ctx *c, const gcnhip_feat *f, const float *vals, const float *w, int ld_w,
                         float *out, int ld_out, int p) {
    return spmm_fwd_impl(c, f, vals, w, ld_w, out, ld_out, p, 0.f, 0, nullptr, 0, nullptr, 1);
}

int gcnhip_spmm_fwd_relu_matmul(gcnhip_ctx *c, const gcnhip_feat *f, const float *vals, const float *w, int ld_w, int p,
                                const float *w2, int ld_w2, int p2, float *z0, int ld_z0) {
    if (!w2 || !z0 || p2 <= 0) return -1;
    const Z0Fuse zf = {w2, ld_w2, p2, z0, ld_z0};
    return spmm_fwd_impl(c, f, vals, w, ld_w, nullptr, 0, p, 0.f, 0, nullptr, 0, nullptr, 1, &zf);
}

static bool dense_bwd_plan(const gcnhip_ctx *c, const gcnhip_feat *f, int p, int *rps_out, int *S_out) {
    if (!(f->dense && p > 64 && f->n_cols >= 64)) return false;
    const int kt = ceil_div(f->n_cols, 128), pt = ceil_div(p, 128);
    int S = (2 * c->n_cu) / (kt * pt);
    if (S < 1) S = 1;
    int rps = (ceil_div(f->n_rows, S) + T_BK - 1) / T_BK * T_BK;
    if (rps < T_BK) rps = T_BK;
    *rps_out = rps;
    *S_out = ceil_div(f->n_rows, rps);
    return true;
}
static bool dense_bwd_bf16x3_fits(const gcnhip_ctx *c, const gcnhip_feat *f, const float *vals, const float *dout, int ld_dout, int p,
                                  const DropSpec &d, int rps) {
    const int bx = c->opt.gemm_bf16x3, kt = ceil_div(f->n_cols, 128);
    const bool padded = vals == f->values && f->values_pad && f->ld_pad >= kt * 128;
    return bx && (bx >= 2 || !c->corun) && p == 128 && padded && rps % 16 == 0 && ld_dout % 4 == 0 && aligned16(dout) &&
           (uint64_t)f->n_rows * (uint64_t)f->ld_pad * 4u < (1ull << 32) && (uint64_t)f->n_rows * (uint64_t)ld_dout * 4u < (1ull << 32) &&
           (uint64_t)f->n_rows * (uint64_t)f->n_cols < (1ull << 32) && (uint64_t)kt * 16u * (uint64_t)f->n_rows < (1ull << 32) &&
           (!d.on || keep_bits_cm_fit(f));
}

static int dense_bwd_part(gcnhip_ctx *c, const gcnhip_feat *f, const float *vals, const float *dout, int ld_dout, int p,
                          const DropSpec &d, int s0, int s1, bool fresh) {
    int rps, S;
    if (!dense_bwd_plan(c, f, p, &rps, &S) || s0 < 0 || s1 > S || s0 > s1) return -1;
    if (s0 == s1) return 0;
    if (d.on && !f->keep_bits) return gcnhip_fail("input dropout on a feature object without a keep-bit array");
    c->slab_n = S;
    const int kt = ceil_div(f->n_cols, 128), pt = ceil_div(p, 128);
    const int p_ld = (p + 3) / 4 * 4;
    const int rc = ensure_slab(c, (size_t)S * f->n_cols * p_ld * sizeof(float));
    if (rc) return rc;
    if (dense_bwd_bf16x3_fits(c, f, vals, dout, ld_dout, p, d, rps)) {
        { const int rl = want_keep_layout(c, f, d, 1, fresh); if (rl) return rl; }
        Bx3BwdArgs b;
        b.x = f->values_pad; b.ldx = f->ld_pad; b.dout = dout; b.ldd = ld_dout; b.slab = c->slab; b.p_ld = p_ld;
        b.m = f->n_rows; b.K = f->n_cols; b.rps = rps; b.split0 = s0; b.bits = d.on ? f->keep_bits : nullptr; b.scale = d.on ? d.scale : 1.f;
        const dim3 grid(kt, s1 - s0);
        if (b.bits) dense_bwd_bf16x3_kernel<true, 6><<<grid, 256, 0, c->stream>>>(b);
        else dense_bwd_bf16x3_kernel<false, 6><<<grid, 256, 0, c->stream>>>(b);
        GCNHIP_LAUNCH_CHECK();
        return 0;
    }
    { const int rl = want_keep_layout(c, f, d, 0, fresh); if (rl) return rl; }
    Tile128Args t;
    t.x = vals; t.ldx = f->n_cols; t.w = dout; t.ldw = ld_dout; t.out = c->slab; t.ldo = p_ld;
    int vx = x_vec_width(f, vals);
    if (vals == f->values && f->values_pad) { t.x = f->values_pad; t.ldx = f->ld_pad; vx = 4; }
    t.m = f->n_rows; t.K = f->n_cols; t.p = p; t.bits = d.on ? f->keep_bits : nullptr; t.scale = d.scale; t.rows_per_split = rps; t.relu = 0;
    t.split0 = s0;
    dim3 grid(s1 - s0, kt, pt);
    const bool fast = vx == 4 && t.ldx % 4 == 0 && kt * 128 <= t.ldx && ld_dout % 4 == 0 && p % 128 == 0 && aligned16(dout);
    if (fast) dense_bwd_t128_kernel<4, true><<<grid, 256, 0, c->stream>>>(t);
    else if (vx == 4) dense_bwd_t128_kernel<4><<<grid, 256, 0, c->stream>>>(t);
    else if (vx == 2) dense_bwd_t128_kernel<2><<<grid, 256, 0, c->stream>>>(t);
    else dense_bwd_t128_kernel<1><<<grid, 256, 0, c->stream>>>(t);
    GCNHIP_LAUNCH_CHECK();
    return 0;
}

static int dense_bwd_finish(gcnhip_ctx *c, const gcnhip_feat *f, float *dw, int ld_dw, int p) {
// ... 106 lines not shown
```

cuda_gcn_amd/host/gcn.h:

```cpp
#pragma once
#include <memory>
#include <utility>
#include <vector>
#include "comm.h"
#include "device_arena.h"
#include "module.h"
#include "optim.h"
#include "partition.h"
#include "sparse.h"
#include "timer.h"
#include "variable.h"

struct GCNParams {
    int num_nodes, input_dim, hidden_dim, output_dim;
    float dropout, learning_rate, weight_decay;
    int epochs, early_stopping;
    static GCNParams get_default();
};

class GCNData {
public:
    SparseIndex feature_index, graph;
    std::vector<int> split;
    std::vector<int> label;
    std::vector<float> feature_value;
    std::vector<uint32_t> multihot;
};

enum HipGCNFlags {
    HIPGCN_MODULAR = 1,
    HIPGCN_HOST_MASKS = 2,
    HIPGCN_TIMERS = 4,
    HIPGCN_NO_GRAPH = 8,
    HIPGCN_EVAL_LANE = 16,
    HIPGCN_NO_EVAL_LANE = 32,
    HIPGCN_NO_REPLICATE_L1 = 64,
    HIPGCN_REPLICATE_L1 = 128,
    HIPGCN_GATHER_DH1 = 256,
    HIPGCN_BF16_TABLES = 2048,
    HIPGCN_ALL_ROWS = 4096,
    HIPGCN_NO_AGG_FIRST_EVAL = 8192,
    HIPGCN_EXCHANGE_ALLGATHER = 16384,
    HIPGCN_EXCHANGE_HALO = 32768,
    HIPGCN_NO_LABEL_HINT = 524288,
    HIPGCN_MASKED_BWD = 131072,
    HIPGCN_NULL_COMM = 1024,
    HIPGCN_NO_ROW_GROUPS = 512,
    HIPGCN_OVERLAP_EXCHANGE = 1048576,
    HIPGCN_STRUCTURE_PARTITION = 2097152,
    HIPGCN_ID_PARTITION = 4194304,
    HIPGCN_EDGE_COEF = 16777216,
    HIPGCN_SYNC_EPOCHS = 8388608,
};

struct HipGCNOptions {
    int device = 0;
    long seed = 0;
    int flags = 0;
    Comm *comm = nullptr;
    bool own_comm = false;
    int rank = 0, world = 1;
    const char *nccl_id = nullptr;
    gcn_host_allgather_fn host_allgather = nullptr;
    gcn_host_allreduce_fn host_allreduce = nullptr;
    void *host_user = nullptr;

    bool verbose = false;
    int exchange = -1;
    bool structure_groups = true;
    bool eval_fusion = true;
    bool loss_epilogue = true;
    bool mask_bits = true;
    bool loss_records_metrics = true;
    bool readback_stream = false;
    int readback_group = 0;
    int schedule = -1, schedule_groups = 256;
    bool slice_tuning = true;
    int gemm = -1;
    bool multilabel = false;
    std::vector<float> class_weights;

    static HipGCNOptions from_environment(HipGCNOptions base);
};

class ModelQueries;

struct ScoredSplit {
    int32_t *truth = nullptr;
    int count = 0;
    float wsum = 0.f;
    gcnhip_rowset *out_rows = nullptr;
    gcnhip_rowset *out_rows_loc = nullptr, *out_rows_rem = nullptr;
    int32_t *rows = nullptr; int rows_n = 0;
};

class HipGCN {
public:
    GCNParams params;
    HipGCN(GCNParams params, GCNData *data, const HipGCNOptions &opt = HipGCNOptions());
    ~HipGCN();
    HipGCN(const HipGCN &) = delete;

    void run();
    std::pair<float, float> train_epoch();
    std::pair<float, float> eval(int current_split);
    void run_epochs(int n, float *trace);
    void sync();

    int rank() const { return env.comm->rank(); }
    int schedule_mode() const { return sched_mode; }
    int schedule_groups() const { return sched_groups; }
    int schedule_slice_floats() const { return slice_floats; }
    int world() const { return env.comm->size(); }
    const char *transport() const { return env.comm->transport(); }
    int transport_ranks() const { return env.comm->transport_ranks(); }
    int local_rows() const { return n_local; }
    int row_start() const { return part.start[env.comm->rank()]; }
    const RowPartition &partition() const { return part; }
    const std::vector<int> &node_order() const { return node_order_; }
    int node_id(int local_row) const { const int p = row_start() + local_row; return node_order_.empty() ? p : node_order_[p]; }
    const char *node_order_name() const { return node_order_name_; }
    const ExchangePlan &exchange_plan() const { return xplan; }
    void get_var(int k, bool grad, std::vector<float> &out, int *rows, int *cols);
    bool factored() const { return factored_; }
    void row_scale(std::vector<float> &dinv);
    void set_weights(const float *w1, const float *w2);
    ModelQueries &queries() { return *queries_; }
    bool multilabel() const { return opt_.multilabel; }
    bool weighted() const { return !opt_.class_weights.empty(); }
    void save_weights(const char *path);
    void load_weights(const char *path);
    DeviceTimers &device_timers() { return *timers; }
    double timer_total(timer_instance t, long *count);
    void timers_reset();
    void set_timers(bool on);
    long n_edges_local() const { return nnzA_local; }

private:
    GCNData *data;
    std::unique_ptr<GCNData> renumbered;
    std::vector<int> node_order_;
    const char *node_order_name_ = "ids";
    void renumber_nodes(int world);
    HipEnv env;
    DeviceArena arena;
    std::unique_ptr<Comm> owned_comm;
    std::unique_ptr<DeviceTimers> timers;
    RowPartition part;
    ExchangePlan xplan;
    ExchangeBuffers xbuf;
    int n_local = 0;
    long nnzA_local = 0;
    int flags = 0;
    bool factored_ = false;
// ... 146 lines not shown
```

cuda_gcn_amd/host/gcn_build.cpp:

```cpp
#include "gcn.h"
#include "queries.h"
#include "class_weights.h"
#include "cluster.h"
#include <chrono>
#include <future>
#include <cstdio>
#include "hip_check.h"

GCNParams GCNParams::get_default() { return {2708, 1433, 16, 7, 0.5, 0.01, 5e-4, 100, 0}; }

namespace {
bool labels_are_assortative(const GCNData &d, int N, int C) {
    if ((int)d.label.size() != N || C <= 1) return false;
    const std::vector<int> &gp = d.graph.indptr, &gi = d.graph.indices;
    std::vector<double> freq(C, 0.0);
    for (int i = 0; i < N; i++) {
        if (d.label[i] < 0 || d.label[i] >= C) return false;
        freq[d.label[i]] += 1.0;
    }
    double chance = 0;
    for (int c = 0; c < C; c++) chance += (freq[c] / N) * (freq[c] / N);
    long same = 0, total = 0;
    for (int i = 0; i < N; i++)
        for (int e = gp[i]; e < gp[i + 1]; e++) {
// ... 280 lines not shown
        std::vector<uint32_t> bits((size_t)n_local / 32 + 2, 0u);
        for (int r = 0; r < n_local; r++)
            if (data->split[r0 + r] == s) bits[r >> 5] |= 1u << (r & 31);
        GCNHIP_CHECK(gcnhip_graph_add_rowset(ctx, g, bits.data(), &out[s]));
    }
}

void HipGCN::build_overlap() {
    const size_t n_pos = (size_t)xplan.table_rows;
    std::vector<uint32_t> own(n_pos / 32 + 2, 0u), other(n_pos / 32 + 2, 0u);
    for (size_t t = 0; t < n_pos; t++) {
        const bool mine = (int)t >= xplan.own_offset && (int)t < xplan.own_offset + n_local;
        (mine ? own : other)[t >> 5] |= 1u << (t & 31);
    }
    xlane.reset(new ExchangeLane(env.ctx, device_, env.comm, xplan, (int)xbuf.max_ld_words, timers->enabled));
    env.xlane = xlane.get();
    if (n_local == 0) return;
    GCNHIP_CHECK(gcnhip_graph_create_restricted(env.ctx, &graph_loc, graph, own.data()));
    GCNHIP_CHECK(gcnhip_graph_create_restricted(env.ctx, &graph_rem, graph, other.data()));
    if (graph_bwd_out) {
        GCNHIP_CHECK(gcnhip_graph_create_restricted(env.ctx, &graph_bwd_loc, graph_bwd_out, own.data()));
        GCNHIP_CHECK(gcnhip_graph_create_restricted(env.ctx, &graph_bwd_rem, graph_bwd_out, other.data()));
    }
    if (!(flags & HIPGCN_ALL_ROWS)) {
        add_split_rowsets(env.ctx, graph_loc, split_rows_loc);
        add_split_rowsets(env.ctx, graph_rem, split_rows_rem);
    }
}

void HipGCN::wire_overlap(HipGraphSum *gs, bool output_layer) {
    if (!graph_loc) return;
    gs->split_loc = graph_loc; gs->split_rem = graph_rem;
    if (!output_layer) return;
    gs->bwd_split_loc = graph_bwd_loc; gs->bwd_split_rem = graph_bwd_rem;
    if (!(flags & HIPGCN_ALL_ROWS)) { gs->fwd_out_rows_loc = &scored.out_rows_loc; gs->fwd_out_rows_rem = &scored.out_rows_rem; }
}

Module *HipGCN::make_loss(const LossSite &s) {
    const int C = params.output_dim;
    if (opt_.multilabel) {
        auto *bce = new HipBCELoss(s.env, s.Z, d_ml_truth, ml_wpr, &s.split->count, s.d_result, s.d_result_i, C);
        bce->rows_list = &s.split->rows; bce->rows_n = &s.split->rows_n; bce->grad_row_scale = s.grad_row_scale;
        bce->d_pos_weight = d_class_w;
        return bce;
    }
    auto *ce = new HipCrossEntropyLoss(s.env, s.Z, &s.split->truth, &s.split->count, s.d_result, s.d_result_i, C, s.shift_in_place);
    if (s.list_rows) { ce->rows_list = &s.split->rows; ce->rows_n = &s.split->rows_n; }
    ce->grad_row_scale = s.grad_row_scale;
    ce->d_weight = d_class_w; ce->weight_sum = &s.split->wsum;
    if (s.epilogue && !d_class_w && opt_.loss_epilogue && C <= 64 && !s.env->bf16_tables) {
        const size_t n = (size_t)2 * std::max(n_local, 1);
        ce->row_terms = (s.env == &env ? arena : lane->arena).upload(std::vector<float>(n, 0.f).data(), n);
        s.epilogue->loss = ce;
    }
    return ce;
}

void HipGCN::build_modules() {
    const int N = n_local, F = params.input_dim, H = params.hidden_dim, C = params.output_dim;
    const int rank = env.comm->rank();
    const uint64_t nnz_off = (uint64_t)data->feature_index.indptr[part.start[rank]];
    const uint64_t hid_off = (uint64_t)part.start[rank] * H;
    HipVariable *H0 = variables[1].get(), *W1 = variables[2].get(), *H1 = variables[3].get(),
                *Z0 = variables[4].get(), *W2 = variables[5].get(), *Z = variables[6].get();
    const float p = params.dropout;
    static const uint8_t *const no_mask = nullptr;
    if (flags & HIPGCN_MODULAR) {
        modules.push_back(new HipDropout(&env, input, p, KEY_INPUT_DROPOUT, nnz_off, (flags & HIPGCN_HOST_MASKS) ? &env.keep_input : &no_mask));
        modules.push_back(new HipSparseMatmul(&env, &input_vals, W1, H0, feat, N, F, H, 0.f, nnz_off));
        { auto *gs = new HipGraphSum(&env, H0, H1, graph, H); wire_overlap(gs, false); modules.push_back(gs); }
        modules.push_back(new HipReLU(&env, H1));
        modules.push_back(new HipDropout(&env, H1, p, KEY_HIDDEN_DROPOUT, hid_off, (flags & HIPGCN_HOST_MASKS) ? &env.keep_hidden : &no_mask));
        modules.push_back(new HipMatmul(&env, H1, W2, Z0, N, H, C));
        { auto *gs = new HipGraphSum(&env, Z0, Z, graph, C); gs->bwd_row_bits = &bwd_bits; gs->bwd_graph = graph_bwd_out; gs->fwd_out_rows = &scored.out_rows; wire_overlap(gs, true); modules.push_back(gs); logits_gs = gs; }
        modules.push_back(make_loss({&env, Z, &scored, d_result, d_result_i, true, nullptr,
                                     opt_.multilabel || d_class_w != nullptr, nullptr}));
    } else {
        const float scale = 1 / (1 - p);
        auto *sm = new HipSparseMatmul(&env, &input_vals, W1, H0, feat, N, F, H, p, nnz_off);
        auto *gs = new HipGraphSum(&env, H0, H1, graph, H, p, hid_off);
        auto *mm = new HipMatmul(&env, H1, W2, Z0, N, H, C, scale);
        if (replicate_l1) { sm->sp_full = feat_full; sm->vals_full = &full_vals; gs->fwd_graph_replicated = graph_l1; }
        wire_overlap(gs, false);
        if (factored_) {
            const float *dinv_row = nullptr, *dinv2_row = nullptr, *dinv2_col = nullptr;
            GCNHIP_CHECK(gcnhip_graph_scales(graph, &dinv_row, &dinv2_row, nullptr, &dinv2_col));
            gs->fwd_scaling = 2; gs->bwd_scaling = 3;
            mm->da_row_scale = dinv2_row;
            mm->da_row_scale_full = dinv2_col;
        }
        if (env.comm->size() == 1 && H % 32 == 0 && !env.bf16_tables && opt_.mask_bits) {
            const int wpr = H / 32;
            d_pos_bits = arena.upload(std::vector<uint32_t>((size_t)N * wpr, 0u).data(), (size_t)N * wpr);
            gs->mask_bits_out = d_pos_bits;
            mm->mask_bits = d_pos_bits; mm->mask_wpr = wpr;
        }
        if (rebuild_dh1) {
            const int wpr = (H + 31) / 32;
            d_pos_bits = arena.upload(std::vector<uint32_t>((size_t)xplan.table_rows * wpr, 0u).data(), (size_t)xplan.table_rows * wpr);
            gs->pos_bits_full = d_pos_bits; gs->wpr = wpr; gs->out_grad_complete = true;
            mm->pos_bits_full = d_pos_bits; mm->wpr = wpr; mm->all_rows = xplan.table_rows;
        }
        modules.push_back(sm);
        modules.push_back(gs);
        modules.push_back(mm);
        HipGraphSum *gs_logits = nullptr;
        {
            auto *gs = new HipGraphSum(&env, Z0, Z, graph, C);
            gs->bwd_row_bits = &bwd_bits; gs->bwd_graph = graph_bwd_out; gs->fwd_out_rows = &scored.out_rows;
            if (factored_) { gs->fwd_scaling = 1; gs->bwd_scaling = 3; }
            wire_overlap(gs, true);
            modules.push_back(gs);
            gs_logits = gs;
            logits_gs = gs;
        }
        const float *dinv = nullptr;
        if (factored_) GCNHIP_CHECK(gcnhip_graph_scales(graph, &dinv, nullptr, nullptr, nullptr));
        modules.push_back(make_loss({&env, Z, &scored, d_result, d_result_i, false, dinv, true, gs_logits}));
    }
}

gcnhip_graph *HipGCN::create_rows_graph(gcnhip_ctx *ctx) {
    const std::vector<int> &gp = data->graph.indptr, &gi = data->graph.indices;
    const int N = params.num_nodes, r0 = part.start[env.comm->rank()];
    std::vector<int> lp(n_local + 1), deg(N);
    for (int r = 0; r <= n_local; r++) lp[r] = gp[r0 + r] - gp[r0];
    for (int j = 0; j < N; j++) deg[j] = gp[j + 1] - gp[j];
    gcnhip_graph *g = nullptr;
    GCNHIP_CHECK(gcnhip_graph_create(ctx, &g, lp.data(), gi.data() + gp[r0], n_local, N, deg.data()));
    const int rc = gcnhip_graph_reserve_width(ctx, g, std::max(params.hidden_dim, params.output_dim));
    if (rc != 0) gcnhip_graph_destroy(ctx, g);
    GCNHIP_CHECK(rc);
    return g;
}

void HipGCN::build_agg_first_eval() {
    const int world = env.comm->size();
    const int N = params.num_nodes, F = params.input_dim, H = params.hidden_dim;
    if (world == 1) {
        GCNHIP_CHECK(gcnhip_feat_create_aggregated(env.ctx, &feat_agg, graph, feat));
    } else {
        const std::vector<int> &fp = data->feature_index.indptr, &fi = data->feature_index.indices;
        gcnhip_graph *g_all = graph_l1;
        gcnhip_feat *x_all = feat_full;
        try {
            if (!g_all) g_all = create_rows_graph(env.ctx);
            if (!x_all)
                GCNHIP_CHECK(gcnhip_feat_create(env.ctx, &x_all, fp.data(), fi.empty() ? nullptr : fi.data(), data->feature_value.data(), N, F));
            GCNHIP_CHECK(gcnhip_feat_create_aggregated(env.ctx, &feat_agg, g_all, x_all));
        } catch (...) {
            if (g_all && g_all != graph_l1) gcnhip_graph_destroy(env.ctx, g_all);
            if (x_all && x_all != feat_full) gcnhip_feat_destroy(env.ctx, x_all);
            throw;
        }
        if (g_all != graph_l1) gcnhip_graph_destroy(env.ctx, g_all);
        if (x_all != feat_full) gcnhip_feat_destroy(env.ctx, x_all);
    }
    agg_vals = gcnhip_feat_values(feat_agg);
    auto *sm = new HipSparseMatmul(&env, &agg_vals, variables[2].get(), variables[3].get(), feat_agg, n_local, F, H, 0.f, 0);
    sm->relu_out = true;
    if (opt_.eval_fusion && !env.bf16_tables) sm->fuse_next = dynamic_cast<HipMatmul *>(modules[2]);
    eval_modules.push_back(sm);
    for (size_t i = 2; i < modules.size(); i++) eval_modules.push_back(modules[i]);
}

void HipGCN::build_eval_lane() {
// ... 125 lines not shown
```

cuda_gcn_amd/host/module.cpp:

```cpp
#include "module.h"
#include <algorithm>
#include "hip_check.h"

HipMatmul::HipMatmul(HipEnv *env, HipVariable *a, HipVariable *b, HipVariable *c, int m, int n, int p, float s)
    : env(env), a(a), b(b), c(c), m(m), n(n), p(p), fused_bwd_scale(s) {}

bool HipMatmul::fused_eval_forward(gcnhip_feat *sp, const float *vals, HipVariable *w1, int p1) {
    if (p1 != n) return false;
    const int rc = gcnhip_spmm_fwd_relu_matmul(env->ctx, sp, vals, w1->data, w1->ld, p1, b->data, b->ld, p, c->data, c->ld);
    if (rc == GCNHIP_NOT_AVAILABLE) return false;
    GCNHIP_CHECK(rc);
    skip_forward_once = true;
    return true;
}

void HipMatmul::forward(bool) {
    if (skip_forward_once) { skip_forward_once = false; return; }
    env->timers->start(TMR_MATMUL_FW);
    GCNHIP_CHECK(gcnhip_matmul_fwd(env->ctx, a->data, a->ld, b->data, b->ld, c->data, c->ld, m, n, p));
    env->timers->stop(TMR_MATMUL_FW);
}

void HipMatmul::backward() {
    env->timers->start(TMR_MATMUL_BW);
// ... 22 lines not shown
    else
        GCNHIP_CHECK(gcnhip_matmul_bwd(env->ctx, a->data, a->ld, b->data, b->ld, c->grad, c->ld,
                                       a->grad, a->ld, b->grad, b->ld, m, n, p));
    env->timers->stop(TMR_MATMUL_BW);
}

void HipMatmul::rebuild_da(int first, int rows) {
    if (rows <= 0) return;
    GCNHIP_CHECK(gcnhip_matmul_bwd_ex(env->ctx, nullptr, 0, b->data, b->ld, c->full_grad + (size_t)first * c->ld, c->ld,
                                      a->full_grad + (size_t)first * a->ld, a->ld, nullptr, 0, rows, n, p, fused_bwd_scale,
                                      pos_bits_full + (size_t)first * wpr, wpr, da_row_scale_full ? da_row_scale_full + first : nullptr));
}

HipSparseMatmul::HipSparseMatmul(HipEnv *env, const float *const *vals, HipVariable *b, HipVariable *c, gcnhip_feat *sp,
                                 int m, int n, int p, float fd, uint64_t off)
    : env(env), vals(vals), b(b), c(c), sp(sp), m(m), n(n), p(p), fused_dropout(fd), nnz_offset(off) {}

void HipSparseMatmul::forward(bool training) {
    last_training = training;
    if (training) fwd_decisions_valid = fused_dropout > 0.f && !sp_full && !relu_out && gcnhip_feat_is_dense(sp);
    env->timers->start(TMR_SPMATMUL_FW);
    const float pd = training ? fused_dropout : 0.f;
    hidden_not_stored = false;
    if (relu_out) {
        if (training) throw GcnHipFailure(-1, "HipSparseMatmul: the ReLU epilogue is an evaluation-only form");
        if (fuse_next && fuse_next->fused_eval_forward(sp, *vals, b, p)) hidden_not_stored = true;
        else GCNHIP_CHECK(gcnhip_spmm_fwd_relu(env->ctx, sp, *vals, b->data, b->ld, c->data, c->ld, p));
    } else if (sp_full)
        GCNHIP_CHECK(gcnhip_spmm_fwd(env->ctx, sp_full, *vals_full, b->data, b->ld, c->full, c->ld, p, pd,
                                     env->seed ^ KEY_INPUT_DROPOUT, env->d_epoch, 0,
                                     pd > 0.f ? env->keep_input : nullptr));
    else
        GCNHIP_CHECK(gcnhip_spmm_fwd(env->ctx, sp, *vals, b->data, b->ld, c->data, c->ld, p, pd,
                                     env->seed ^ KEY_INPUT_DROPOUT, env->d_epoch, nnz_offset,
                                     pd > 0.f ? env->keep_input : nullptr));
    env->timers->stop(TMR_SPMATMUL_FW);
}

void HipSparseMatmul::forward_stored() {
    if (!relu_out) throw GcnHipFailure(-1, "HipSparseMatmul::forward_stored: an evaluation-only form");
    GCNHIP_CHECK(gcnhip_spmm_fwd_relu(env->ctx, sp, *vals, b->data, b->ld, c->data, c->ld, p));
    hidden_not_stored = false;
}

void HipSparseMatmul::backward() {
    env->timers->start(TMR_SPMATMUL_BW);
    const float pd = last_training ? fused_dropout : 0.f;
    int rps = 0, n_splits = 0;
    GCNHIP_CHECK(gcnhip_spmm_bwd_plan(env->ctx, sp, p, &rps, &n_splits));
    if (n_splits > 0 && pd > 0.f && fwd_decisions_valid) {
        GCNHIP_CHECK(gcnhip_spmm_bwd_part(env->ctx, sp, *vals, c->grad, c->ld, p, pd, env->seed ^ KEY_INPUT_DROPOUT, env->d_epoch,
                                          nnz_offset, env->keep_input_bwd, 0, n_splits, 0));
        GCNHIP_CHECK(gcnhip_spmm_bwd_finish(env->ctx, sp, b->grad, b->ld, p));
    } else {
        GCNHIP_CHECK(gcnhip_spmm_bwd(env->ctx, sp, *vals, c->grad, c->ld, b->grad, b->ld, p, pd,
                                     env->seed ^ KEY_INPUT_DROPOUT, env->d_epoch, nnz_offset,
                                     pd > 0.f ? env->keep_input_bwd : nullptr));
    }
    env->timers->stop(TMR_SPMATMUL_BW);
}

HipGraphSum::HipGraphSum(HipEnv *env, HipVariable *in, HipVariable *out, gcnhip_graph *graph, int dim, float frd, uint64_t off)
    : env(env), in(in), out(out), graph(graph), dim(dim), fused_relu_dropout(frd), elem_offset(off) {}

HipGraphSum::~HipGraphSum() { if (bf_table) gcnhip_free(env->ctx, bf_table); }

size_t HipGraphSum::full_rows(const HipVariable *v, bool grad) {
    const float *full = grad ? v->full_grad : v->full;
    return full ? v->full_elems / v->ld : (size_t)v->rows;
}

uint16_t *HipGraphSum::table() {
    if (!bf_table) {
        ld_bf = dim <= 8 ? 8 : (dim <= 16 ? 16 : (dim <= 32 ? 32 : (dim + 63) / 64 * 64));
        bf_rows = std::max(full_rows(in, false), full_rows(out, true));
        void *p;
        GCNHIP_CHECK(gcnhip_malloc(env->ctx, &p, bf_rows * ld_bf * sizeof(uint16_t)));
        GCNHIP_CHECK(gcnhip_memset_async(env->ctx, p, 0, bf_rows * ld_bf * sizeof(uint16_t)));
        bf_table = (uint16_t *)p;
    }
    return bf_table;
}

void HipGraphSum::forward(bool training) {
    gcnhip_graph *graph = this->graph;
    const int world = env->comm->size();
    const gcnhip_rowset *out_rows = fwd_out_rows ? *fwd_out_rows : nullptr;
    const bool replicated = in->replicated && fwd_graph_replicated;
    if (replicated) graph = fwd_graph_replicated;
    bool bits_written = false;
    if (env->bf16_tables) {
        uint16_t *tab = table();
        env->timers->start(TMR_GRAPHSUM_FW);
        if (replicated) {
            GCNHIP_CHECK(gcnhip_f32_to_bf16(env->ctx, in->full, in->ld, tab, ld_bf, (int64_t)full_rows(in, false), dim));
        } else {
            const size_t own = world > 1 ? (size_t)env->plan->own_offset : 0;
            GCNHIP_CHECK(gcnhip_f32_to_bf16(env->ctx, in->data, in->ld, tab + own * ld_bf, ld_bf, in->rows, dim));
            if (world > 1) {
                env->timers->start(TMR_COMM);
                env->comm->exchange_rows(*env->plan, *env->xbuf, reinterpret_cast<float *>(tab), ld_bf / 2);
                env->timers->stop(TMR_COMM);
            }
        }
        if (dim > 64) env->timers->start(TMR_GRAPHSUM_WIDE);
        const bool fused = fused_relu_dropout >= 0.f;
        if (predict)
            GCNHIP_CHECK(gcnhip_graphsum_predict(env->ctx, graph, predict->rows, nullptr, tab, ld_bf, nullptr, 0, dim, 0, predict->pred,
                                                 predict->prob, predict->logp, predict->ld_logp));
        else
            GCNHIP_CHECK(gcnhip_graphsum_bf16(env->ctx, graph, tab, ld_bf, redirect ? redirect->data : out->data, redirect ? redirect->ld : out->ld, dim,
                                              nullptr, redirect ? redirect->rows : out_rows, fused ? 1 : 0, training ? 1 : 0,
                                              fused ? fused_relu_dropout : 0.f, env->seed ^ KEY_HIDDEN_DROPOUT, env->d_epoch, elem_offset,
                                              training ? env->keep_hidden : nullptr));
        if (dim > 64) env->timers->stop(TMR_GRAPHSUM_WIDE);
        env->timers->stop(TMR_GRAPHSUM_FW);
    } else if (env->xlane && !replicated && world > 1 && !predict && !redirect) {
        void *ev = env->xlane->begin(*env->plan, in->full, in->ld);
        const gcnhip_rowset *rows_loc = fwd_out_rows_loc ? *fwd_out_rows_loc : nullptr, *rows_rem = fwd_out_rows_rem ? *fwd_out_rows_rem : nullptr;
        const bool fused = fused_relu_dropout >= 0.f;
        env->timers->start(TMR_GRAPHSUM_FW);
        if (dim > 64) env->timers->start(TMR_GRAPHSUM_WIDE);
        if (split_loc) {
            gcnhip_gs_opts o1 = {};
            o1.rows = rows_loc; o1.scaling = fwd_scaling ? 3 : 0;
            GCNHIP_CHECK(gcnhip_graphsum_ex(env->ctx, split_loc, &o1, in->full, in->ld, out->data, out->ld, dim));
        }
        env->xlane->wait(ev);
        if (split_loc) {
            gcnhip_gs_opts o2 = {};
            o2.rows = rows_rem; o2.accumulate = 1; o2.scaling = fwd_scaling;
            o2.relu_dropout = fused ? 1 : 0; o2.training = training ? 1 : 0; o2.p = fused ? fused_relu_dropout : 0.f;
            o2.seed = env->seed ^ KEY_HIDDEN_DROPOUT; o2.d_epoch = env->d_epoch; o2.elem_offset = elem_offset;
            o2.keep_mask = training ? env->keep_hidden : nullptr;
            GCNHIP_CHECK(gcnhip_graphsum_ex(env->ctx, split_rem, &o2, in->full, in->ld, out->data, out->ld, dim));
        }
        if (dim > 64) env->timers->stop(TMR_GRAPHSUM_WIDE);
        env->timers->stop(TMR_GRAPHSUM_FW);
    } else {
        if (!replicated && world > 1) {
            env->timers->start(TMR_COMM);
            env->comm->exchange_rows(*env->plan, *env->xbuf, in->full, in->ld);
            env->timers->stop(TMR_COMM);
        }
        const float *src = in->full ? in->full : in->data;
        env->timers->start(TMR_GRAPHSUM_FW);
        if (dim > 64) env->timers->start(TMR_GRAPHSUM_WIDE);
        uint32_t *bits_here = nullptr;
        if (training && fused_relu_dropout >= 0.f && dim % 32 == 0)
            bits_here = mask_bits_out ? mask_bits_out : (pos_bits_full ? pos_bits_full + (size_t)env->plan->own_offset * wpr : nullptr);
        if (predict) {
            GCNHIP_CHECK(gcnhip_graphsum_predict(env->ctx, graph, predict->rows, src, nullptr, in->ld, nullptr, 0, dim, fwd_scaling, predict->pred,
                                                 predict->prob, predict->logp, predict->ld_logp));
        } else {
            gcnhip_gs_opts o = {};
            o.scaling = fwd_scaling;
            if (fused_relu_dropout >= 0.f) {
                o.relu_dropout = 1; o.training = training ? 1 : 0; o.p = fused_relu_dropout;
                o.seed = env->seed ^ KEY_HIDDEN_DROPOUT; o.d_epoch = env->d_epoch; o.elem_offset = elem_offset;
                o.keep_mask = training ? env->keep_hidden : nullptr;
                if (bits_here) { o.pos_bits = bits_here; o.words_per_row = mask_bits_out ? (dim + 31) / 32 : wpr; bits_written = true; }
            } else {
                o.rows = redirect ? redirect->rows : out_rows;
            }
            gcnhip_gs_loss lo = {};
            if (loss && !redirect && fused_relu_dropout < 0.f && loss->epilogue_opts(training, &lo)) { o.loss = &lo; loss->terms_fresh = true; }
            GCNHIP_CHECK(gcnhip_graphsum_ex(env->ctx, graph, &o, src, in->ld, redirect ? redirect->data : out->data, redirect ? redirect->ld : out->ld, dim));
        }
        if (dim > 64) env->timers->stop(TMR_GRAPHSUM_WIDE);
        env->timers->stop(TMR_GRAPHSUM_FW);
    }
    if (pos_bits_full && training) {
        uint32_t *mine = pos_bits_full + (size_t)env->plan->own_offset * wpr;
        if (!bits_written) GCNHIP_CHECK(gcnhip_pack_positive(env->ctx, out->data, out->ld, out->rows, dim, mine, wpr));
        if (env->xlane) {
            if (env->pos_bits_ready) env->xlane->wait(env->pos_bits_ready);
            env->pos_bits_ready = env->xlane->begin(*env->plan, reinterpret_cast<float *>(pos_bits_full), wpr);
        } else {
            env->timers->start(TMR_COMM);
            env->comm->exchange_rows(*env->plan, *env->xbuf, reinterpret_cast<float *>(pos_bits_full), wpr);
            env->timers->stop(TMR_COMM);
        }
    }
}

void HipGraphSum::backward() {
    const int world = env->comm->size();
    const uint32_t *row_bits = bwd_row_bits && !bwd_graph ? *bwd_row_bits : nullptr;
    const gcnhip_graph *graph = bwd_graph ? bwd_graph : this->graph;
    if (env->bf16_tables) {
        uint16_t *tab = table();
        env->timers->start(TMR_GRAPHSUM_BW);
        if (world > 1 && out_grad_complete) {
            GCNHIP_CHECK(gcnhip_f32_to_bf16(env->ctx, out->full_grad, out->ld, tab, ld_bf, (int64_t)full_rows(out, true), dim));
        } else {
            const size_t own = world > 1 ? (size_t)env->plan->own_offset : 0;
            GCNHIP_CHECK(gcnhip_f32_to_bf16(env->ctx, out->grad, out->ld, tab + own * ld_bf, ld_bf, out->rows, dim));
            if (world > 1) {
                env->timers->start(TMR_COMM);
                env->comm->exchange_rows(*env->plan, *env->xbuf, reinterpret_cast<float *>(tab), ld_bf / 2);
                env->timers->stop(TMR_COMM);
            }
        }
        if (dim > 64) env->timers->start(TMR_GRAPHSUM_WIDE);
        GCNHIP_CHECK(gcnhip_graphsum_bf16(env->ctx, graph, tab, ld_bf, in->grad, in->ld, dim, row_bits, nullptr, 0, 0, 0.f, 0, nullptr, 0, nullptr));
        if (dim > 64) env->timers->stop(TMR_GRAPHSUM_WIDE);
        env->timers->stop(TMR_GRAPHSUM_BW);
        return;
    }
    if (world > 1 && !out_grad_complete && env->xlane) {
        const gcnhip_graph *loc = bwd_split_loc ? bwd_split_loc : split_loc, *rem = bwd_split_rem ? bwd_split_rem : split_rem;
        const uint32_t *bits = bwd_split_loc ? nullptr : row_bits;
        void *ev = env->xlane->begin(*env->plan, out->full_grad, out->ld);
        env->timers->start(TMR_GRAPHSUM_BW);
        if (dim > 64) env->timers->start(TMR_GRAPHSUM_WIDE);
        gcnhip_gs_opts o = {};
        o.in_row_bits = bits; o.scaling = bwd_scaling;
        if (loc) GCNHIP_CHECK(gcnhip_graphsum_ex(env->ctx, loc, &o, out->full_grad, out->ld, in->grad, in->ld, dim));
        env->xlane->wait(ev);
        o.accumulate = 1;
        if (rem) GCNHIP_CHECK(gcnhip_graphsum_ex(env->ctx, rem, &o, out->full_grad, out->ld, in->grad, in->ld, dim));
        if (dim > 64) env->timers->stop(TMR_GRAPHSUM_WIDE);
        env->timers->stop(TMR_GRAPHSUM_BW);
        return;
    }
    if (world > 1 && !out_grad_complete) {
        env->timers->start(TMR_COMM);
        env->comm->exchange_rows(*env->plan, *env->xbuf, out->full_grad, out->ld);
        env->timers->stop(TMR_COMM);
    }
    const float *src = out->full_grad ? out->full_grad : out->grad;
    env->timers->start(TMR_GRAPHSUM_BW);
    if (dim > 64) env->timers->start(TMR_GRAPHSUM_WIDE);
    gcnhip_gs_opts o = {};
    o.in_row_bits = row_bits; o.scaling = bwd_scaling;
    GCNHIP_CHECK(gcnhip_graphsum_ex(env->ctx, graph, &o, src, out->ld, in->grad, in->ld, dim));
    if (dim > 64) env->timers->stop(TMR_GRAPHSUM_WIDE);
    env->timers->stop(TMR_GRAPHSUM_BW);
}

HipCrossEntropyLoss::HipCrossEntropyLoss(HipEnv *env, HipVariable *logits, int32_t *const *truth, const int *count,
                                         float *d_result, int32_t *d_result_i, int num_classes, bool shift)
    : env(env), logits(logits), truth(truth), count(count), d_result(d_result), d_result_i(d_result_i),
// ... 86 lines not shown
```

cuda_gcn_amd/host/module.h:

```cpp
#pragma once
#include <vector>
#include <cstdint>
#include "comm.h"
#include "gcnhip_driver.h"
#include "timer.h"
#include "variable.h"

struct HipEnv {
    gcnhip_ctx *ctx = nullptr;
    Comm *comm = nullptr;
    const ExchangePlan *plan = nullptr;
    ExchangeBuffers *xbuf = nullptr;
    DeviceTimers *timers = nullptr;
    uint64_t seed = 0;
    uint32_t *d_epoch = nullptr;
    uint32_t *d_epoch_done = nullptr;
    const uint8_t *keep_input = nullptr;
    const uint8_t *keep_input_bwd = nullptr;
    const uint8_t *keep_hidden = nullptr;
    bool bf16_tables = false;
    ExchangeLane *xlane = nullptr;
    void *pos_bits_ready = nullptr;
};

class Module {
public:
    virtual void forward(bool) = 0;
    virtual void backward() = 0;
    virtual ~Module() {}
};

class HipMatmul : public Module {
    HipEnv *env;
    HipVariable *a, *b, *c;
    int m, n, p;
    float fused_bwd_scale;
public:
    const uint32_t *pos_bits_full = nullptr;
    int wpr = 0, all_rows = 0;
    const uint32_t *mask_bits = nullptr;
    int mask_wpr = 0;
    const float *da_row_scale = nullptr, *da_row_scale_full = nullptr;
    HipMatmul(HipEnv *env, HipVariable *a, HipVariable *b, HipVariable *c, int m, int n, int p, float fused_bwd_scale = 0.f);
    bool fused_eval_forward(gcnhip_feat *sp, const float *vals, HipVariable *w1, int p1);
private:
    bool skip_forward_once = false;
    void rebuild_da(int first_row, int n_rows);
public:
    void forward(bool) override;
    void backward() override;
};

class HipSparseMatmul : public Module {
    HipEnv *env;
    const float *const *vals;
    HipVariable *b, *c;
    gcnhip_feat *sp;
    int m, n, p;
    float fused_dropout;
    uint64_t nnz_offset;
    bool last_training = false;
    bool fwd_decisions_valid = false;
public:
    gcnhip_feat *sp_full = nullptr;
    const float *const *vals_full = nullptr;
    bool relu_out = false;
    HipMatmul *fuse_next = nullptr;
    bool hidden_not_stored = false;
    void forward_stored();
    HipSparseMatmul(HipEnv *env, const float *const *vals, HipVariable *b, HipVariable *c, gcnhip_feat *sp,
                    int m, int n, int p, float fused_dropout, uint64_t nnz_offset);
    void forward(bool) override;
    void backward() override;
};

class HipCrossEntropyLoss;
class HipGraphSum : public Module {
    HipEnv *env;
    HipVariable *in, *out;
    gcnhip_graph *graph;
    int dim;
    float fused_relu_dropout;
    uint64_t elem_offset;
public:
    HipCrossEntropyLoss *loss = nullptr;
    gcnhip_graph *fwd_graph_replicated = nullptr;
    uint32_t *pos_bits_full = nullptr;
    int wpr = 0;
    bool out_grad_complete = false;
    uint32_t *mask_bits_out = nullptr;
    const uint32_t *const *bwd_row_bits = nullptr;
    const gcnhip_graph *bwd_graph = nullptr;
    gcnhip_rowset *const *fwd_out_rows = nullptr;
    const gcnhip_graph *split_loc = nullptr, *split_rem = nullptr;
    const gcnhip_graph *bwd_split_loc = nullptr, *bwd_split_rem = nullptr;
    gcnhip_rowset *const *fwd_out_rows_loc = nullptr, *const *fwd_out_rows_rem = nullptr;
    int fwd_scaling = 0, bwd_scaling = 0;
    struct Prediction {
        const gcnhip_rowset *rows = nullptr;
        int32_t *pred = nullptr;
        float *prob = nullptr, *logp = nullptr;
        int ld_logp = 0;
    };
    const Prediction *predict = nullptr;
    struct Redirect {
        float *data = nullptr;
        int ld = 0;
        const gcnhip_rowset *rows = nullptr;
    };
    const Redirect *redirect = nullptr;
    HipGraphSum(HipEnv *env, HipVariable *in, HipVariable *out, gcnhip_graph *graph, int dim,
                float fused_relu_dropout = -1.f, uint64_t elem_offset = 0);
    ~HipGraphSum() override;
    void forward(bool) override;
    void backward() override;
private:
    uint16_t *bf_table = nullptr;
    int ld_bf = 0;
    size_t bf_rows = 0;
    uint16_t *table();
    static size_t full_rows(const HipVariable *v, bool grad);
};

class HipCrossEntropyLoss : public Module {
    HipEnv *env;
    HipVariable *logits;
    int32_t *const *truth;
    const int *count;
    float *d_result;
    int32_t *d_result_i;
    int num_classes;
    bool shift_in_place;
public:
    int32_t *const *rows_list = nullptr;
    const int *rows_n = nullptr;
    const float *grad_row_scale = nullptr;
    float *row_terms = nullptr;
    bool terms_fresh = false;
    bool epilogue_opts(bool training, gcnhip_gs_loss *o) const;
    const float *d_weight = nullptr;
    const float *weight_sum = nullptr;
    HipCrossEntropyLoss(HipEnv *env, HipVariable *logits, int32_t *const *truth, const int *count,
                        float *d_result, int32_t *d_result_i, int num_classes, bool shift_in_place);
    void forward(bool) override;
    void backward() override {}
};

class HipBCELoss : public Module {
    HipEnv *env;
    HipVariable *logits;
    const uint32_t *truth;
    int wpr;
    const int *count;
    float *d_result;
    int32_t *d_result_i;
    int num_classes;
public:
    int32_t *const *rows_list = nullptr;
    const int *rows_n = nullptr;
    const float *grad_row_scale = nullptr;
    const float *d_pos_weight = nullptr;
    HipBCELoss(HipEnv *env, HipVariable *logits, const uint32_t *truth, int wpr, const int *count,
               float *d_result, int32_t *d_result_i, int num_classes);
    void forward(bool) override;
    void backward() override {}
};

class HipReLU : public Module {
    HipEnv *env;
    HipVariable *in;
    uint8_t *mask;
public:
    HipReLU(HipEnv *env, HipVariable *in);
    ~HipReLU() override;
    void forward(bool) override;
    void backward() override;
};

class HipDropout : public Module {
    HipEnv *env;
    HipVariable *in;
    int32_t *mask;
    float p;
    uint64_t key_tweak, elem_offset;
    const uint8_t *const *keep_in;
public:
    HipDropout(HipEnv *env, HipVariable *in, float p, uint64_t key_tweak, uint64_t elem_offset, const uint8_t *const *keep_in);
    ~HipDropout() override;
    void forward(bool) override;
    void backward() override;
};

constexpr uint64_t KEY_INPUT_DROPOUT = 0x9E3779B97F4A7C15ull;
constexpr uint64_t KEY_HIDDEN_DROPOUT = 0xD1B54A32D192ED03ull;
```

cuda_gcn_amd/host/options.cpp:

```cpp
#include <cstdlib>
#include <cstring>
#include "gcn.h"

HipGCNOptions HipGCNOptions::from_environment(HipGCNOptions o) {
    static const struct { const char *name; int bit; } flag_vars[] = {
        {"HIPGCN_EDGE_COEF", HIPGCN_EDGE_COEF},
        {"HIPGCN_STRUCTURE_PARTITION", HIPGCN_STRUCTURE_PARTITION},
        {"HIPGCN_ID_PARTITION", HIPGCN_ID_PARTITION},
        {"HIPGCN_NO_LABEL_HINT", HIPGCN_NO_LABEL_HINT},
        {"HIPGCN_ALL_ROWS", HIPGCN_ALL_ROWS},
        {"HIPGCN_MASKED_BWD", HIPGCN_MASKED_BWD},
        {"HIPGCN_OVERLAP_EXCHANGE", HIPGCN_OVERLAP_EXCHANGE},
        {"HIPGCN_NO_AGG_FIRST_EVAL", HIPGCN_NO_AGG_FIRST_EVAL},
        {"HIPGCN_EVAL_LANE", HIPGCN_EVAL_LANE},
        {"HIPGCN_SYNC_EPOCHS", HIPGCN_SYNC_EPOCHS},
    };
    for (const auto &f : flag_vars)
        if (getenv(f.name)) o.flags |= f.bit;
    if (getenv("HIPGCN_VERBOSE")) o.verbose = true;
    if (const char *e = getenv("HIPGCN_EXCHANGE"))
        o.exchange = !strcmp(e, "halo") ? 2 : (!strcmp(e, "allgather") ? 1 : (!strcmp(e, "auto") ? 0 : o.exchange));
    if (getenv("HIPGCN_NO_STRUCTURE_GROUPS")) o.structure_groups = false;
    if (getenv("HIPGCN_NO_MASK_BITS")) o.mask_bits = false;
    if (getenv("HIPGCN_NO_LOSS_EPILOGUE")) o.loss_epilogue = false;
    if (getenv("HIPGCN_NO_EVAL_FUSION")) o.eval_fusion = false;
    if (getenv("HIPGCN_NO_SLICE_TUNING")) o.slice_tuning = false;
    if (getenv("HIPGCN_RECORD_LAUNCH")) o.loss_records_metrics = false;
    if (const char *e = getenv("HIPGCN_READBACK_STREAM")) o.readback_stream = atoi(e) != 0;
    if (const char *e = getenv("HIPGCN_READBACK_GROUP")) o.readback_group = atoi(e);
    if (const char *e = getenv("HIPGCN_SCHEDULE")) {
        if (!strcmp(e, "degree")) o.schedule = 0;
        else if (!strcmp(e, "label")) o.schedule = 1;
        else if (!strncmp(e, "dealt", 5)) { o.schedule = 2; if (e[5] == '-' && atoi(e + 6) > 0) o.schedule_groups = atoi(e + 6); }
        else if (!strcmp(e, "structure")) o.schedule = 3;
    }
    if (const char *e = getenv("HIPGCN_GEMM")) o.gemm = !strcmp(e, "bf16x3") ? 1 : (!strcmp(e, "f32") ? 0 : o.gemm);
    return o;
}
```

cuda_gcn_amd/ops.py:

```python
from __future__ import annotations

import ctypes as C

import numpy as np

from . import _lib


class GsOpts(C.Structure):
    _fields_ = [("rows", C.c_void_p), ("in_row_bits", C.c_void_p), ("accumulate", C.c_int), ("relu_dropout", C.c_int), ("training", C.c_int),
                ("p", C.c_float), ("seed", C.c_uint64), ("d_epoch", C.c_void_p), ("elem_offset", C.c_uint64), ("keep_mask", C.c_void_p),
                ("pos_bits", C.c_void_p), ("words_per_row", C.c_int), ("scaling", C.c_int), ("loss", C.c_void_p)]


class GsLoss(C.Structure):
    _fields_ = [("truth", C.c_void_p), ("grad", C.c_void_p), ("ld_grad", C.c_int), ("training", C.c_int), ("count", C.c_int),
                ("grad_row_scale", C.c_void_p), ("row_terms", C.c_void_p)]


class GcnHipError(RuntimeError):
    pass


def _ck(lib, code, what):
    if code != 0:
        msg = lib.gcnhip_error_string(code)
        raise GcnHipError(f"{what}: error {code} ({msg.decode() if msg else '?'})")


class Buf:

    def __init__(self, dev: "Device", shape, dtype):
        self.dev = dev
        self.shape = tuple(int(s) for s in np.atleast_1d(shape))
        self.dtype = np.dtype(dtype)
        self.nbytes = int(np.prod(self.shape)) * self.dtype.itemsize
        p = C.c_void_p()
        _ck(dev.lib, dev.lib.gcnhip_malloc(dev.ctx, C.byref(p), max(self.nbytes, 16)), "gcnhip_malloc")
        self.ptr = p.value

    def upload(self, arr):
        arr = np.ascontiguousarray(arr, self.dtype)
        assert arr.nbytes == self.nbytes, (arr.shape, self.shape)
        _ck(self.dev.lib, self.dev.lib.gcnhip_h2d(self.dev.ctx, self.ptr, arr.ctypes.data, self.nbytes), "gcnhip_h2d")
        return self

    def download(self):
        out = np.empty(self.shape, self.dtype)
        _ck(self.dev.lib, self.dev.lib.gcnhip_d2h(self.dev.ctx, out.ctypes.data, self.ptr, self.nbytes), "gcnhip_d2h")
        return out

    def fill_bytes(self, byte=0):
        _ck(self.dev.lib, self.dev.lib.gcnhip_memset_async(self.dev.ctx, self.ptr, byte, self.nbytes), "memset")
        return self

    def free(self):
        if self.ptr and self.dev.ctx:
            self.dev.lib.gcnhip_free(self.dev.ctx, self.ptr)
        self.ptr = None

    def __del__(self):
        try:
            self.free()
        except Exception:
            pass


class Device:

    def __init__(self, device: int = 0, stream=None):
        self.lib = _lib.gcnhip()
        n = C.c_int()
        _ck(self.lib, self.lib.gcnhip_device_count(C.byref(n)), "gcnhip_device_count")
        if n.value <= device:
            raise GcnHipError(f"no GPU {device} (device count {n.value}); this package has no CPU path")
        ctx = C.c_void_p()
        _ck(self.lib, self.lib.gcnhip_ctx_create(C.byref(ctx), device, stream), "gcnhip_ctx_create")
        self.ctx = ctx

    def close(self):
        if self.ctx:
            self.lib.gcnhip_ctx_destroy(self.ctx)
            self.ctx = None

    def sync(self):
        _ck(self.lib, self.lib.gcnhip_ctx_sync(self.ctx), "sync")

    def set_option(self, name: str, value: int):
        _ck(self.lib, self.lib.gcnhip_ctx_set_option(self.ctx, name.encode(), int(value)), f"gcnhip_ctx_set_option({name})")

    def get_option(self, name: str) -> int:
        v = C.c_int()
        _ck(self.lib, self.lib.gcnhip_ctx_get_option(self.ctx, name.encode(), C.byref(v)), f"gcnhip_ctx_get_option({name})")
        return v.value

# ... 274 lines not shown
        x = np.asarray(x, np.float32)
        dim = x.shape[1]
        ld_in = ld_in or dim
        ld_out = ld_out or dim
        xin = self.padded(x, ld_in)
        out = self.buf(np.full((g.n_rows, ld_out), np.nan, np.float32))
        g.reserve(dim)
        if row_nonzero is None:
            _ck(self.lib, self.lib.gcnhip_graphsum(self.ctx, g.h, xin.ptr, ld_in, out.ptr, ld_out, dim), "gcnhip_graphsum")
        else:
            bits = np.packbits(np.asarray(row_nonzero, bool), bitorder="little")
            bits = np.concatenate([bits, np.zeros((-bits.size) % 4 + 4, np.uint8)]).view(np.uint32)
            bb = self.buf(bits)
            _ck(self.lib, self.lib.gcnhip_graphsum_rowmask(self.ctx, g.h, xin.ptr, ld_in, out.ptr, ld_out, dim, bb.ptr), "gcnhip_graphsum_rowmask")
        return out.download()[:, :dim]

    def gather_rows(self, x, rows):
        x = np.ascontiguousarray(x, np.float32)
        rows = np.ascontiguousarray(rows, np.int32)
        xb, rb = self.buf(x), self.buf(rows if rows.size else np.zeros(1, np.int32))
        out = self.buf(np.full((max(rows.size, 1), x.shape[1]), np.nan, np.float32))
        _ck(self.lib, self.lib.gcnhip_gather_rows(self.ctx, xb.ptr, x.shape[1], rb.ptr, int(rows.size), out.ptr), "gcnhip_gather_rows")
        return out.download()[:rows.size]

    def to_bf16(self, x, ld_dst=None):
        x = np.asarray(x, np.float32)
        rows, dim = x.shape
        ld_dst = ld_dst or (dim + 7) // 8 * 8
        xb = self.buf(np.ascontiguousarray(x))
        dst = self.buf(np.full((rows, ld_dst), 0xFFFF, np.uint16))
        _ck(self.lib, self.lib.gcnhip_f32_to_bf16(self.ctx, xb.ptr, dim, dst.ptr, ld_dst, rows, dim), "gcnhip_f32_to_bf16")
        return dst.download()

    def graphsum_bf16(self, g: "Graph", table_u16, dim, ld_out=None, row_nonzero=None, relu_dropout=None, out_rows=None, fill=np.nan):
        t = np.ascontiguousarray(table_u16, np.uint16)
        ld_in = t.shape[1]
        ld_out = ld_out or dim
        tb = self.buf(t)
        out = self.buf(np.full((g.n_rows, ld_out), fill, np.float32))
        bb = None
        if row_nonzero is not None:
            bits = np.packbits(np.asarray(row_nonzero, bool), bitorder="little")
            bits = np.concatenate([bits, np.zeros((-bits.size) % 4 + 4, np.uint8)]).view(np.uint32)
            bb = self.buf(bits)
        rd = relu_dropout or {}
        g.reserve(dim)
        ep = self.buf(np.array([rd.get("epoch", 0)], np.uint32))
        km = self.buf(np.ascontiguousarray(rd["keep_mask"], np.uint8)) if rd.get("keep_mask") is not None else None
        _ck(self.lib, self.lib.gcnhip_graphsum_bf16(self.ctx, g.h, tb.ptr, ld_in, out.ptr, ld_out, dim, bb.ptr if bb else None,
                                                     out_rows,
                                                     1 if relu_dropout is not None else 0, int(rd.get("training", 0)), float(rd.get("p", 0.0)),
                                                     int(rd.get("seed", 0)), ep.ptr, int(rd.get("elem_offset", 0)), km.ptr if km else None),
            "gcnhip_graphsum_bf16")
        return out.download()[:, :dim]

    def graphsum_relu_dropout(self, g, x, training, p, seed=0, epoch=0, elem_offset=0, keep_mask=None, ld=None):
        x = np.asarray(x, np.float32)
        dim = x.shape[1]
        ld = ld or dim
        xin = self.padded(x, ld)
        out = self.buf(np.full((g.n_rows, ld), np.nan, np.float32))
        g.reserve(dim)
        ep = self.buf(np.array([epoch], np.uint32))
        km = self.buf(np.ascontiguousarray(keep_mask, np.uint8)) if keep_mask is not None else None
        _ck(self.lib, self.lib.gcnhip_graphsum_relu_dropout(self.ctx, g.h, xin.ptr, ld, out.ptr, ld, dim, int(training), p,
                                                             seed, ep.ptr, elem_offset, km.ptr if km else None), "graphsum_relu_dropout")
        return out.download()[:, :dim]

    def graphsum_relu_dropout_bits(self, g, x, training, p, seed=0, epoch=0, elem_offset=0, keep_mask=None, ld=None):
        x = np.asarray(x, np.float32)
        dim = x.shape[1]
        ld = ld or dim
        wpr = (dim + 31) // 32
        xin = self.padded(x, ld)
        out = self.buf(np.full((g.n_rows, ld), np.nan, np.float32))
        bits = self.buf(np.full((g.n_rows, wpr), 0xDEADBEEF, np.uint32))
        g.reserve(dim)
        ep = self.buf(np.array([epoch], np.uint32))
        km = self.buf(np.ascontiguousarray(keep_mask, np.uint8)) if keep_mask is not None else None
        _ck(self.lib, self.lib.gcnhip_graphsum_relu_dropout_bits(self.ctx, g.h, xin.ptr, ld, out.ptr, ld, dim, int(training), p, seed, ep.ptr,
                                                                  elem_offset, km.ptr if km else None, bits.ptr, wpr), "graphsum_relu_dropout_bits")
        return out.download()[:, :dim], bits.download()

    def matmul_bwd_fused_bits(self, a, b, dc, scale, bits):
        a, b, dc = (np.asarray(t, np.float32) for t in (a, b, dc))
        m, n = a.shape
        p = b.shape[1]
        ldp = (p + 3) // 4 * 4
        ab, bb, dcb = self.buf(a), self.padded(b, ldp), self.padded(dc, ldp)
        bt = self.buf(np.ascontiguousarray(bits, np.uint32))
        da = self.buf(np.full((m, n), np.nan, np.float32))
        db = self.buf(np.full((n, ldp), np.nan, np.float32))
        _ck(self.lib, self.lib.gcnhip_matmul_bwd_fused_bits(self.ctx, ab.ptr, n, bb.ptr, ldp, dcb.ptr, ldp, da.ptr, n, db.ptr, ldp, m, n, p, scale,
                                                             bt.ptr, bits.shape[1]), "gcnhip_matmul_bwd_fused_bits")
        return da.download(), db.download()[:, :p]

    def matmul_bwd_ex(self, a, b, dc, scale, bits, rowscale=None, ldp=None, p=None):
        a, b, dc = (np.asarray(t, np.float32) for t in (a, b, dc))
        m, n = a.shape
        p = p or b.shape[1]
        ldp = ldp or (p + 3) // 4 * 4
        ab, bb, dcb = self.buf(a), self.padded(b, ldp), self.padded(dc, ldp)
        bt = self.buf(np.ascontiguousarray(bits, np.uint32))
        rs = self.buf(np.ascontiguousarray(rowscale, np.float32)) if rowscale is not None else None
        da = self.buf(np.full((m, n), np.nan, np.float32))
        db = self.buf(np.full((n, ldp), np.nan, np.float32))
        _ck(self.lib, self.lib.gcnhip_matmul_bwd_ex(self.ctx, ab.ptr, n, bb.ptr, ldp, dcb.ptr, ldp, da.ptr, n, db.ptr, ldp, m, n, p, scale,
                                                     bt.ptr, bits.shape[1], rs.ptr if rs else None), "gcnhip_matmul_bwd_ex")
        return da.download(), db.download()[:, :p]

    def spmm_fwd(self, f: "Feat", w, p_drop=0.0, seed=0, epoch=0, nnz_offset=0, keep_mask=None, vals=None, ld_w=None, ld_out=None):
        w = np.asarray(w, np.float32)
        p = w.shape[1]
        ld_w = ld_w or p
        ld_out = ld_out or p
        wb = self.padded(w, ld_w)
        out = self.buf(np.full((f.n_rows, ld_out), np.nan, np.float32))
        ep = self.buf(np.array([epoch], np.uint32))
        km = self.buf(np.ascontiguousarray(keep_mask, np.uint8)) if keep_mask is not None else None
        vb = self.buf(np.ascontiguousarray(vals, np.float32)) if vals is not None else None
        vptr = vb.ptr if vb else f.values_ptr
        _ck(self.lib, self.lib.gcnhip_spmm_fwd(self.ctx, f.h, vptr, wb.ptr, ld_w, out.ptr, ld_out, p, p_drop, seed, ep.ptr,
                                                nnz_offset, km.ptr if km else None), "gcnhip_spmm_fwd")
        return out.download()[:, :p]

    def spmm_fwd_relu(self, f: "Feat", w, ld_w=None, ld_out=None):
        w = np.asarray(w, np.float32)
        p = w.shape[1]
        ld_w, ld_out = ld_w or p, ld_out or p
        wb = self.padded(w, ld_w)
        out = self.buf(np.full((f.n_rows, ld_out), np.nan, np.float32))
        _ck(self.lib, self.lib.gcnhip_spmm_fwd_relu(self.ctx, f.h, f.values_ptr, wb.ptr, ld_w, out.ptr, ld_out, p), "gcnhip_spmm_fwd_relu")
        return out.download()[:, :p]

    def spmm_fwd_relu_matmul(self, f: "Feat", w, w2, ld_z=None):
        w, w2 = np.asarray(w, np.float32), np.asarray(w2, np.float32)
        p, p2 = w.shape[1], w2.shape[1]
        ld_z = ld_z or (p2 + 3) // 4 * 4
        wb, w2b = self.buf(w), self.padded(w2, ld_z)
        z = self.buf(np.full((f.n_rows, ld_z), np.nan, np.float32))
        rc = self.lib.gcnhip_spmm_fwd_relu_matmul(self.ctx, f.h, f.values_ptr, wb.ptr, p, p, w2b.ptr, ld_z, p2, z.ptr, ld_z)
        if rc == -2:
            return None
        _ck(self.lib, rc, "gcnhip_spmm_fwd_relu_matmul")
        return z.download()[:, :p2]

    def spmm_bwd(self, f: "Feat", dout, p_drop=0.0, seed=0, epoch=0, nnz_offset=0, keep_mask=None, vals=None, ld_dout=None, ld_dw=None):
        dout = np.asarray(dout, np.float32)
        p = dout.shape[1]
        ld_dout = ld_dout or p
        ld_dw = ld_dw or p
        db = self.padded(dout, ld_dout)
        dw = self.buf(np.full((f.n_cols, ld_dw), np.nan, np.float32))
        ep = self.buf(np.array([epoch], np.uint32))
        km = self.buf(np.ascontiguousarray(keep_mask, np.uint8)) if keep_mask is not None else None
        vb = self.buf(np.ascontiguousarray(vals, np.float32)) if vals is not None else None
        vptr = vb.ptr if vb else f.values_ptr
        _ck(self.lib, self.lib.gcnhip_spmm_bwd(self.ctx, f.h, vptr, db.ptr, ld_dout, dw.ptr, ld_dw, p, p_drop, seed, ep.ptr,
                                                nnz_offset, km.ptr if km else None), "gcnhip_spmm_bwd")
        return dw.download()[:, :p]

    def spmm_bwd_plan(self, f: "Feat", p):
        rps, ns = C.c_int(), C.c_int()
        _ck(self.lib, self.lib.gcnhip_spmm_bwd_plan(self.ctx, f.h, p, C.byref(rps), C.byref(ns)), "gcnhip_spmm_bwd_plan")
        return rps.value, ns.value

# ... 485 lines not shown
```

include/gcnhip_driver.h:

```cpp
#ifndef GCNHIP_DRIVER_H
#define GCNHIP_DRIVER_H
#include "gcnhip.h"
#ifdef __cplusplus
extern "C" {
#endif

typedef struct gcnhip_rowset gcnhip_rowset;

int gcnhip_ctx_set_corun(gcnhip_ctx *ctx, int on);
int gcnhip_host_alloc(void **ptr, size_t bytes);
int gcnhip_host_free(void *ptr);
int gcnhip_d2h_async(gcnhip_ctx *ctx, void *dst_pinned, const void *src, size_t bytes);
int gcnhip_graph_create_grouped(gcnhip_ctx *ctx, gcnhip_graph **g, const int *h_indptr, const int *h_indices,
                                int n_rows, int n_cols, const int *h_col_deg, const int *h_row_group);
int gcnhip_graph_set_schedule(gcnhip_ctx *ctx, gcnhip_graph *g, int mode, const int *h_row_group, int n_groups);
int gcnhip_graphsum_rowmask(gcnhip_ctx *ctx, const gcnhip_graph *g, const float *in, int ld_in,
                            float *out, int ld_out, int dim, const uint32_t *in_row_bits);
int gcnhip_graphsum_masked(gcnhip_ctx *ctx, const gcnhip_graph *g, const float *in, int ld_in,
                           float *out, int ld_out, int dim, const uint32_t *in_row_bits, const uint32_t *out_row_bits);
int gcnhip_graph_add_rowset(gcnhip_ctx *ctx, gcnhip_graph *g, const uint32_t *h_row_bits, gcnhip_rowset **rows);
int gcnhip_rowset_size(const gcnhip_rowset *rows, int *n_tasks);
int gcnhip_graphsum_rowset(gcnhip_ctx *ctx, const gcnhip_graph *g, const gcnhip_rowset *rows, const float *in, int ld_in,
                           float *out, int ld_out, int dim, const uint32_t *in_row_bits);
int gcnhip_graph_create_restricted(gcnhip_ctx *ctx, gcnhip_graph **out, const gcnhip_graph *parent, const uint32_t *h_col_bits);
int gcnhip_graph_clone(gcnhip_ctx *ctx, gcnhip_graph **out, const gcnhip_graph *parent);
int gcnhip_graphsum_part(gcnhip_ctx *ctx, const gcnhip_graph *g, const gcnhip_rowset *rows, const float *in, int ld_in,
                         float *out, int ld_out, int dim, const uint32_t *in_row_bits, int accumulate,
                         int relu_dropout, int training, float p, uint64_t seed, const uint32_t *d_epoch,
                         uint64_t elem_offset, const uint8_t *keep_mask);
int gcnhip_graphsum_relu_dropout(gcnhip_ctx *ctx, const gcnhip_graph *g, const float *in, int ld_in,
                                 float *out, int ld_out, int dim, int training, float p,
                                 uint64_t seed, const uint32_t *d_epoch, uint64_t elem_offset,
                                 const uint8_t *keep_mask);
int gcnhip_graphsum_relu_dropout_bits(gcnhip_ctx *ctx, const gcnhip_graph *g, const float *in, int ld_in,
                                      float *out, int ld_out, int dim, int training, float p,
                                      uint64_t seed, const uint32_t *d_epoch, uint64_t elem_offset,
                                      const uint8_t *keep_mask, uint32_t *pos_bits, int words_per_row);
typedef struct {
    const gcnhip_rowset *rows;
    const uint32_t *in_row_bits;
    int accumulate;
    int relu_dropout, training;
    float p;
    uint64_t seed;
    const uint32_t *d_epoch;
    uint64_t elem_offset;
    const uint8_t *keep_mask;
    uint32_t *pos_bits;
    int words_per_row;
    int scaling;
    const struct gcnhip_gs_loss *loss;
} gcnhip_gs_opts;
typedef struct gcnhip_gs_loss {
    const int32_t *truth;
    float *grad; int ld_grad;
    int training, count;
    const float *grad_row_scale;
    float *row_terms;
} gcnhip_gs_loss;
int gcnhip_graphsum_ex(gcnhip_ctx *ctx, const gcnhip_graph *g, const gcnhip_gs_opts *opts, const float *in, int ld_in,
                       float *out, int ld_out, int dim);
int gcnhip_graphsum_predict(gcnhip_ctx *ctx, const gcnhip_graph *g, const gcnhip_rowset *rows, const float *in, const uint16_t *in_bf16,
                            int ld_in, float *out, int ld_out, int dim, int scaling, int32_t *pred, float *prob, float *logp, int ld_logp);
int gcnhip_graphsum_blend(gcnhip_ctx *ctx, const gcnhip_graph *g, const float *in, int ld_in, const float *base, int ld_base,
                          float *out, int ld_out, int dim, float alpha, float beta, float lo, float hi, int32_t *pred);
int gcnhip_cs_error_rows(gcnhip_ctx *ctx, const float *logp, int ld_logp, const int32_t *truth, int n_table, const int32_t *d_rows,
                         int n_listed, int num_classes, float *e, int ld_e, float *d_sigma);
int gcnhip_cs_correct_rows(gcnhip_ctx *ctx, const float *logp, int ld_logp, const float *e_hat, int ld_e, const int32_t *truth, int n_table,
                           int num_classes, const float *d_sigma, float *g0, int ld_g);
int gcnhip_calib_nll_rows(gcnhip_ctx *ctx, const float *logp, int ld, const int32_t *truth, int n_table, const int32_t *d_rows, int n,
                          int num_classes, float beta, double *d_out);
int gcnhip_calib_bins_rows(gcnhip_ctx *ctx, const float *logp, int ld, const int32_t *truth, int n_table, const int32_t *d_rows, int n,
                           int num_classes, float beta, int bins, int32_t *d_count, int32_t *d_correct, double *d_conf_sum);
int gcnhip_calib_scale_rows(gcnhip_ctx *ctx, const float *logp, int ld, int n_table, const int32_t *d_rows, int n, int num_classes, float beta,
                            float *out_logp, int ld_out, float *d_prob);
int gcnhip_embed_inv_norms(gcnhip_ctx *ctx, const float *table, int ld, int n_table, int dim, float *inv_norm);
int gcnhip_topk_plan(int n_table, int nq, int k, int chunk_rows, int *chunk_rows_used, int *n_chunks, size_t *scratch_bytes,
                     size_t *scratch_bytes_min);
int gcnhip_topk_rows(gcnhip_ctx *ctx, const float *table, int ld, int n_table, int dim, const float *inv_norm, const int32_t *row_id,
                     const int32_t *q_rows, int nq, int k, int exclude_self, int chunk_rows, void *scratch, size_t scratch_bytes,
                     int launches, int32_t *out_id, float *out_score);
int gcnhip_pair_scores(gcnhip_ctx *ctx, const float *table, int ld, int n_table, int dim, const float *inv_norm, const int32_t *src,
                       const int32_t *dst, int n_pairs, float *out);
int gcnhip_embed_rows(gcnhip_ctx *ctx, const float *table, int ld, int n_table, int dim, const float *inv_norm, const int32_t *d_rows,
                      int n, float *out, int ld_out);
int gcnhip_graph_remove_rowset(gcnhip_ctx *ctx, gcnhip_graph *g, gcnhip_rowset *rows);
int gcnhip_graph_scales(const gcnhip_graph *g, const float **d_dinv_row, const float **d_dinv2_row,
                        const float **d_dinv_col, const float **d_dinv2_col);
int gcnhip_feat_scale_rows(gcnhip_ctx *ctx, gcnhip_feat *f, const float *d_row_scale);

int gcnhip_feat_create_aggregated(gcnhip_ctx *ctx, gcnhip_feat **f, gcnhip_graph *g, const gcnhip_feat *x);
int gcnhip_spmm_fwd_relu(gcnhip_ctx *ctx, const gcnhip_feat *f, const float *vals, const float *w, int ld_w,
                         float *out, int ld_out, int p);
#define GCNHIP_NOT_AVAILABLE (-2)
int gcnhip_spmm_fwd_relu_matmul(gcnhip_ctx *ctx, const gcnhip_feat *f, const float *vals, const float *w, int ld_w, int p,
                                const float *w2, int ld_w2, int p2, float *z0, int ld_z0);
int gcnhip_spmm_bwd_plan(const gcnhip_ctx *ctx, const gcnhip_feat *f, int p, int *rows_per_split, int *n_splits);
int gcnhip_spmm_bwd_part(gcnhip_ctx *ctx, const gcnhip_feat *f, const float *vals, const float *dout, int ld_dout, int p,
                         float p_drop, uint64_t seed, const uint32_t *d_epoch, uint64_t nnz_offset, const uint8_t *keep_mask,
                         int split_begin, int split_end, int make_decisions);
int gcnhip_spmm_bwd_finish(gcnhip_ctx *ctx, const gcnhip_feat *f, float *dw, int ld_dw, int p);

int gcnhip_f32_to_bf16(gcnhip_ctx *ctx, const float *src, int ld_src, uint16_t *dst, int ld_dst, int64_t rows, int dim);
int gcnhip_graphsum_bf16(gcnhip_ctx *ctx, const gcnhip_graph *g, const uint16_t *in_bf16, int ld_in,
                         float *out, int ld_out, int dim, const uint32_t *in_row_bits, const gcnhip_rowset *out_rows,
                         int relu_dropout, int training, float p, uint64_t seed, const uint32_t *d_epoch,
                         uint64_t elem_offset, const uint8_t *keep_mask);

int gcnhip_matmul_bwd_fused(gcnhip_ctx *ctx, const float *a, int lda, const float *b, int ldb,
                            const float *dc, int lddc, float *da, int ldda, float *db, int lddb,
                            int m, int n, int p, float relu_dropout_scale);
int gcnhip_matmul_bwd_fused_bits(gcnhip_ctx *ctx, const float *a, int lda, const float *b, int ldb,
                                 const float *dc, int lddc, float *da, int ldda, float *db, int lddb,
                                 int m, int n, int p, float relu_dropout_scale, const uint32_t *pos_bits, int words_per_row);

int gcnhip_matmul_bwd_ex(gcnhip_ctx *ctx, const float *a, int lda, const float *b, int ldb,
                         const float *dc, int lddc, float *da, int ldda, float *db, int lddb,
                         int m, int n, int p, float relu_dropout_scale, const uint32_t *pos_bits, int words_per_row,
                         const float *d_da_row_scale);

int gcnhip_pack_positive(gcnhip_ctx *ctx, const float *h, int ld, int n_rows, int dim, uint32_t *bits, int words_per_row);
int gcnhip_matmul_bwd_da_bits(gcnhip_ctx *ctx, const float *b, int ldb, const float *dc, int lddc,
                              float *da, int ldda, int m, int n, int p,
                              const uint32_t *h_pos_bits, int words_per_row, float scale);

int gcnhip_gather_rows(gcnhip_ctx *ctx, const float *src, int ld_words, const int *d_rows, int n, float *dst);

int gcnhip_relu_dropout_bwd(gcnhip_ctx *ctx, float *grad, int ld_grad, const float *h, int ld_h,
                            int n_rows, int dim, float scale);

int gcnhip_xent_fwd_rows(gcnhip_ctx *ctx, float *logits, int ld, float *grad, int ld_grad,
                         const int32_t *truth, const int32_t *d_rows, int n_listed, int num_classes, int training,
                         int count, int shift_in_place, float *d_result, int32_t *d_result_i);
int gcnhip_xent_fwd_rows_scaled(gcnhip_ctx *ctx, float *logits, int ld, float *grad, int ld_grad,
                                const int32_t *truth, const int32_t *d_rows, int n_listed, int num_classes, int training,
// ... 43 lines not shown
```

Measured before the change: 348.1.

## Precompute hidden dropout keep bits and skip idle wave iterations in bf16x3 GEMM

```diff
diff --git a/cuda_gcn_amd/_lib.py b/cuda_gcn_amd/_lib.py
--- a/cuda_gcn_amd/_lib.py
+++ b/cuda_gcn_amd/_lib.py
@@ -96,6 +96,7 @@
     "gcnhip_graphsum_relu_dropout": (I, [P, P, P, I, P, I, I, I, F, U64, P, U64, P]),
     "gcnhip_graphsum_relu_dropout_bits": (I, [P, P, P, I, P, I, I, I, F, U64, P, U64, P, P, I]),
     "gcnhip_graphsum_ex": (I, [P, P, P, P, I, P, I, I]),
+    "gcnhip_keep_words": (I, [P, P, I64, F, U64, P, U64]),
     "gcnhip_graphsum_predict": (I, [P, P, P, P, P, I, P, I, I, I, P, P, P, I]),
     "gcnhip_graphsum_blend": (I, [P, P, P, I, P, I, P, I, I, F, F, F, F, P]),
     "gcnhip_cs_error_rows": (I, [P, P, I, P, I, P, I, I, P, I, P]),
diff --git a/cuda_gcn_amd/csrc/dense_bf16x3.h b/cuda_gcn_amd/csrc/dense_bf16x3.h
--- a/cuda_gcn_amd/csrc/dense_bf16x3.h
+++ b/cuda_gcn_amd/csrc/dense_bf16x3.h
@@ -187,12 +187,12 @@
         for (int r = 0; r < 16; r++) acc[n][r] = 0.f;
 
     const __amdgpu_buffer_rsrc_t orsrc = __builtin_amdgcn_make_buffer_rsrc(a.out, 0, (int)((uint32_t)a.m * (uint32_t)a.ldo * 4u), 0x00020000);
-    auto store_block = [&](f32x16 &v, int row0, int col, bool live) __attribute__((always_inline)) {
+    auto store_block = [&](f32x16 &v, int row0, int col) __attribute__((always_inline)) {
 #pragma unroll
         for (int r = 0; r < 16; r++) {
             const int row = row0 + (r & 3) + 8 * (r >> 2) + 4 * hh;
             const float x = (a.relu && !(v[r] > 0.f)) ? 0.f : v[r];
-            const uint32_t off = live ? ((uint32_t)row * (uint32_t)a.ldo + (uint32_t)col) * 4u : 0xFFFFFFF0u;
+            const uint32_t off = ((uint32_t)row * (uint32_t)a.ldo + (uint32_t)col) * 4u;
             __builtin_amdgcn_raw_buffer_store_b32(__float_as_uint(x), orsrc, (int)off, 0, 0);
             v[r] = 0.f;
         }
@@ -238,7 +238,7 @@
         c = MFMA_BF16(ah, B.m, c);
         c = MFMA_BF16(ah, B.h, c);
     };
-    auto second_product = [&](int row0, bool live) __attribute__((always_inline)) {
+    auto second_product = [&](int row0) __attribute__((always_inline)) {
         const uint4 *img = reinterpret_cast<const uint4 *>(smem + NBV * BX_BH_BYTES);
         f32x16 z[2];
 #pragma unroll
@@ -276,7 +276,7 @@
 #pragma unroll
             for (int r = 0; r < 16; r++) acc[n][r] = 0.f;
         const int row = row0 + li;
-        if (live && row < a.m) {
+        if (row < a.m) {
             float *zp = a.z0 + (size_t)row * a.ldz;
 #pragma unroll
             for (int cb = 0; cb < 2; cb++)
@@ -406,24 +406,33 @@
         __builtin_amdgcn_sched_barrier(0);
         BX_WAIT_LDS(Bc);
         if (c == a.n_chunks - 1) {
-            const bool live = 8 * t + wave < nb;
             if (ZOUT) {
-                second_product((rb_lo + 8 * t + wave) * 32, live);
+                second_product((rb_lo + 8 * t + wave) * 32);
             } else {
 #pragma unroll
-                for (int n = 0; n < 4; n++) store_block(acc[n], (rb_lo + 8 * t + wave) * 32, 32 * n + li, live);
+                for (int n = 0; n < 4; n++) store_block(acc[n], (rb_lo + 8 * t + wave) * 32, 32 * n + li);
             }
         }
     };
+    const int n_live = (wave < nb ? (nb - wave + 7) / 8 : 0) * a.n_chunks;
     int g = 0;
-    for (; g + 3 <= n_items; g += 3) {
+    for (; g + 3 <= n_live; g += 3) {
         chunk(R0, R1, R2, g);
         chunk(R1, R2, R0, g + 1);
         chunk(R2, R0, R1, g + 2);
     }
+    if (g < n_live) {
+        chunk(R0, R1, R2, g); g++;
+        if (g < n_live) { chunk(R1, R2, R0, g); g++; }
+    }
     if (g < n_items) {
-        chunk(R0, R1, R2, g); g++;
-        if (g < n_items) { chunk(R1, R2, R0, g); g++; }
+        BX_WAIT_RAW(0, R0);
+        BX_WAIT_RAW(0, R1);
+        BX_WAIT_RAW(0, R2);
+        for (int h = 2 * g; h < 2 * n_items; h++) {
+            BX_WAIT_W();
+            issue_b(h + BX_PD);
+        }
     }
     BX_WAIT_RAW(0, R0);
     BX_WAIT_RAW(0, R1);
@@ -554,6 +563,34 @@
 #pragma unroll
         for (int r = 0; r < 16; r++) acc[n][r] = 0.f;
 
+    if (n_steps > 0 && F0 >= a.K) {
+        BxRaw8 Q0, Q1;
+        BxPlanes PB;
+        load_raw(Q0, 0);
+        load_raw(Q1, 1);
+        if (DROP) BX_WAIT_RAW8(17, Q0); else BX_WAIT_RAW8(16, Q0);
+#pragma unroll
+        for (int i = 0; i < 4; i++) split_b_pair(PB, Q0, i);
+        write_b(PB, 0);
+        asm volatile("s_waitcnt lgkmcnt(0)\n\ts_barrier" ::: "memory");
+        auto step = [&](BxRaw8 &Rn, BxRaw8 &Rf, int s) __attribute__((always_inline)) {
+            load_raw(Rf, s + 2);
+            if (DROP) BX_WAIT_RAW8(17, Rn); else BX_WAIT_RAW8(16, Rn);
+#pragma unroll
+            for (int i = 0; i < 4; i++) split_b_pair(PB, Rn, i);
+            write_b(PB, (s & 1) ^ 1);
+            asm volatile("s_waitcnt lgkmcnt(0)\n\ts_barrier" ::: "memory");
+        };
+        int s = 0;
+        for (; s + 2 <= n_steps; s += 2) {
+            step(Q1, Q0, s);
+            step(Q0, Q1, s + 1);
+        }
+        if (s < n_steps) step(Q1, Q0, s);
+        BX_WAIT_RAW8(0, Q0);
+        BX_WAIT_RAW8(0, Q1);
+        return;
+    }
     if (n_steps > 0) {
         BxRaw8 R0, R1;
         load_raw(R0, 0);
diff --git a/cuda_gcn_amd/csrc/graphsum.hip b/cuda_gcn_amd/csrc/graphsum.hip
--- a/cuda_gcn_amd/csrc/graphsum.hip
+++ b/cuda_gcn_amd/csrc/graphsum.hip
@@ -20,6 +20,8 @@
     uint64_t seed, elem_offset;
     const uint32_t *d_epoch;
     const uint8_t *keep_mask;
+    const uint32_t *keep_words;
+    uint64_t keep_bit0;
     const uint32_t *row_bits;
     const uint32_t *out_bits;
     uint32_t *pos_bits;
@@ -46,6 +48,21 @@
     return make_float4(__shfl_xor(v.x, m, WAVE), __shfl_xor(v.y, m, WAVE), __shfl_xor(v.z, m, WAVE), __shfl_xor(v.w, m, WAVE));
 }
 
+__device__ inline uint32_t keep4_words(const GsArgs &a, uint64_t j) {
+    const uint64_t rel = j - a.keep_bit0;
+    const uint32_t *w = a.keep_words + (rel >> 5);
+    const uint32_t sh = (uint32_t)rel & 31u;
+    uint32_t bits = w[0] >> sh;
+    if (sh > 28u) bits |= w[1] << (32u - sh);
+    return bits & 15u;
+}
+__device__ inline bool keep_elem(const GsArgs &a, int64_t e) {
+    if (a.keep_mask) return a.keep_mask[e] != 0;
+    const uint64_t j = a.elem_offset + (uint64_t)e;
+    if (a.keep_words) return keep4_words(a, j) & 1u;
+    return keep1(j, a.d_epoch ? *a.d_epoch : 0u, a.seed, a.thr);
+}
+
 __device__ inline float4 relu_dropout4(float4 v, const GsArgs &a, int64_t r, int col0) {
     float x[4] = {v.x, v.y, v.z, v.w};
 #pragma unroll
@@ -60,7 +77,9 @@
             for (int i = 0; i < 4; i++) bits |= (col0 + i < a.dim && a.keep_mask[e0 + i] ? 1u : 0u) << i;
         } else {
             const uint64_t j0 = a.elem_offset + (uint64_t)e0;
-            if ((j0 & 3) == 0) {
+            if (a.keep_words) {
+                bits = keep4_words(a, j0);
+            } else if ((j0 & 3) == 0) {
                 bits = keep4(j0 >> 2, epoch, a.seed, a.thr);
             } else {
                 bits = 0;
@@ -678,8 +697,7 @@
                         v = v > 0.f ? v : 0.f;
                         if (a.training) {
                             const int64_t e = (int64_t)row * a.dim + col;
-                            const bool keep = a.keep_mask ? a.keep_mask[e] != 0
-                                                          : keep1(a.elem_offset + (uint64_t)e, a.d_epoch ? *a.d_epoch : 0u, a.seed, a.thr);
+                            const bool keep = keep_elem(a, e);
                             v *= keep ? a.scale : 0.f;
                         }
                     }
@@ -720,8 +738,7 @@
                 v = v > 0.f ? v : 0.f;
                 if (a.training) {
                     const int64_t e = (int64_t)row * a.dim + col;
-                    const bool keep = a.keep_mask ? a.keep_mask[e] != 0
-                                                  : keep1(a.elem_offset + (uint64_t)e, a.d_epoch ? *a.d_epoch : 0u, a.seed, a.thr);
+                    const bool keep = keep_elem(a, e);
                     v *= keep ? a.scale : 0.f;
                 }
             }
@@ -908,7 +925,8 @@
                          uint64_t elem_offset, const uint8_t *keep_mask, const uint32_t *row_bits = nullptr,
                          const uint16_t *in_bf = nullptr, const uint32_t *out_bits = nullptr,
                          const gcnhip_rowset *rs = nullptr, int accumulate = 0, uint32_t *pos_bits = nullptr, int wpr = 0, int scaling = 0,
-                         const gcnhip_gs_loss *loss = nullptr, const PredArgs *pred = nullptr) {
+                         const gcnhip_gs_loss *loss = nullptr, const PredArgs *pred = nullptr,
+                         const uint32_t *keep_words = nullptr, uint64_t keep_bit0 = 0) {
     if (!c || !g || (!in && !in_bf) || (!out && !pred) || dim <= 0 || ld_in < dim || ld_out < dim) return -1;
     if (scaling < 0 || scaling > 3) return -1;
     if (accumulate && in_bf) return -1;
@@ -931,6 +949,7 @@
     a.fuse = fuse; a.training = training; a.thr = dropout_threshold(p);
     a.scale = 1 / (1 - p);
     a.seed = seed; a.elem_offset = elem_offset; a.d_epoch = d_epoch; a.keep_mask = keep_mask;
+    a.keep_words = (fuse && training && !keep_mask) ? keep_words : nullptr; a.keep_bit0 = keep_bit0;
     a.row_bits = row_bits;
     a.out_bits = out_bits;
     a.accumulate = accumulate;
@@ -1053,9 +1072,11 @@
     if (!o) return -1;
     if (o->relu_dropout && o->training && !(o->p >= 0.f && o->p < 1.f)) return -1;
     if (o->pos_bits && !o->relu_dropout) return -1;
+    if (o->keep_words && (o->keep_bit0 > o->elem_offset || ((uintptr_t)o->keep_words & 3)))
+        return gcnhip_fail("gcnhip_graphsum_ex: keep_words start at stream bit keep_bit0 <= elem_offset (gcnhip_keep_words)");
     return graphsum_impl(c, g, in, ld_in, out, ld_out, dim, o->relu_dropout ? 1 : 0, o->relu_dropout ? o->training : 0, o->relu_dropout ? o->p : 0.f,
                          o->seed, o->d_epoch, o->elem_offset, o->keep_mask, o->in_row_bits, nullptr, nullptr, o->rows, o->accumulate ? 1 : 0,
-                         o->pos_bits, o->words_per_row, o->scaling, o->loss);
+                         o->pos_bits, o->words_per_row, o->scaling, o->loss, nullptr, o->keep_words, o->keep_bit0);
 }
 
 int gcnhip_graphsum_predict(gcnhip_ctx *c, const gcnhip_graph *g, const gcnhip_rowset *rows, const float *in, const uint16_t *in_bf16,
diff --git a/cuda_gcn_amd/csrc/spmm.hip b/cuda_gcn_amd/csrc/spmm.hip
--- a/cuda_gcn_amd/csrc/spmm.hip
+++ b/cuda_gcn_amd/csrc/spmm.hip
@@ -357,6 +357,15 @@
     if (units <= 1) SPF(1); else if (units <= 2) SPF(2); else if (units <= 4) SPF(4);
     else if (units <= 8) SPF(8); else if (units <= 16) SPF(16); else if (units <= 32) SPF(32); else SPF(64);
 #undef SPF
+    GCNHIP_LAUNCH_CHECK();
+    return 0;
+}
+
+int gcnhip_keep_words(gcnhip_ctx *c, uint32_t *words, int64_t n_bits, float p, uint64_t seed, const uint32_t *d_epoch, uint64_t bit0) {
+    if (!c || !words || n_bits < 0 || !(p >= 0.f && p < 1.f) || (bit0 & 127) || !aligned16(words)) return -1;
+    if (n_bits == 0) return 0;
+    const int64_t blocks = (n_bits + 127) / 128;
+    dropbits_block_kernel<<<(unsigned)((blocks + 255) / 256), 256, 0, c->stream>>>(words, n_bits, dropout_threshold(p), seed, d_epoch, bit0 >> 7);
     GCNHIP_LAUNCH_CHECK();
     return 0;
 }
diff --git a/cuda_gcn_amd/host/gcn.h b/cuda_gcn_amd/host/gcn.h
--- a/cuda_gcn_amd/host/gcn.h
+++ b/cuda_gcn_amd/host/gcn.h
@@ -70,6 +70,7 @@
     bool structure_groups = true;
     bool eval_fusion = true;
     bool loss_epilogue = true;
+    bool hidden_keep_words = true;
     bool mask_bits = true;
     bool loss_records_metrics = true;
     bool readback_stream = false;
diff --git a/cuda_gcn_amd/host/gcn_build.cpp b/cuda_gcn_amd/host/gcn_build.cpp
--- a/cuda_gcn_amd/host/gcn_build.cpp
+++ b/cuda_gcn_amd/host/gcn_build.cpp
@@ -386,6 +386,10 @@
         auto *mm = new HipMatmul(&env, H1, W2, Z0, N, H, C, scale);
         if (replicate_l1) { sm->sp_full = feat_full; sm->vals_full = &full_vals; gs->fwd_graph_replicated = graph_l1; }
         wire_overlap(gs, false);
+        if (opt_.hidden_keep_words && !(flags & HIPGCN_HOST_MASKS) && !env.bf16_tables && p > 0.f && N > 0) {
+            const size_t words = HipGraphSum::keep_words_needed(hid_off, (size_t)N, H, &gs->keep_words_bits);
+            gs->keep_words = arena.alloc<uint32_t>(words + 4);
+        }
         if (factored_) {
             const float *dinv_row = nullptr, *dinv2_row = nullptr, *dinv2_col = nullptr;
             GCNHIP_CHECK(gcnhip_graph_scales(graph, &dinv_row, &dinv2_row, nullptr, &dinv2_col));
diff --git a/cuda_gcn_amd/host/module.cpp b/cuda_gcn_amd/host/module.cpp
--- a/cuda_gcn_amd/host/module.cpp
+++ b/cuda_gcn_amd/host/module.cpp
@@ -128,6 +128,18 @@
     return bf_table;
 }
 
+size_t HipGraphSum::keep_words_needed(uint64_t elem_offset, size_t rows, int dim, int64_t *n_bits) {
+    const int64_t bits = (int64_t)(elem_offset & 127) + (int64_t)rows * dim + 32;
+    if (n_bits) *n_bits = bits;
+    return (size_t)((bits + 127) / 128 * 4);
+}
+
+void HipGraphSum::draw_keep_words(gcnhip_gs_opts *o) {
+    const uint64_t bit0 = elem_offset & ~(uint64_t)127;
+    GCNHIP_CHECK(gcnhip_keep_words(env->ctx, keep_words, keep_words_bits, fused_relu_dropout, env->seed ^ KEY_HIDDEN_DROPOUT, env->d_epoch, bit0));
+    o->keep_words = keep_words; o->keep_bit0 = bit0;
+}
+
 void HipGraphSum::forward(bool training) {
     gcnhip_graph *graph = this->graph;
     const int world = env->comm->size();
@@ -179,6 +191,7 @@
             o2.relu_dropout = fused ? 1 : 0; o2.training = training ? 1 : 0; o2.p = fused ? fused_relu_dropout : 0.f;
             o2.seed = env->seed ^ KEY_HIDDEN_DROPOUT; o2.d_epoch = env->d_epoch; o2.elem_offset = elem_offset;
             o2.keep_mask = training ? env->keep_hidden : nullptr;
+            if (fused && training && keep_words && !env->keep_hidden) draw_keep_words(&o2);
             GCNHIP_CHECK(gcnhip_graphsum_ex(env->ctx, split_rem, &o2, in->full, in->ld, out->data, out->ld, dim));
         }
         if (dim > 64) env->timers->stop(TMR_GRAPHSUM_WIDE);
@@ -205,6 +218,7 @@
                 o.relu_dropout = 1; o.training = training ? 1 : 0; o.p = fused_relu_dropout;
                 o.seed = env->seed ^ KEY_HIDDEN_DROPOUT; o.d_epoch = env->d_epoch; o.elem_offset = elem_offset;
                 o.keep_mask = training ? env->keep_hidden : nullptr;
+                if (training && keep_words && !env->keep_hidden) draw_keep_words(&o);
                 if (bits_here) { o.pos_bits = bits_here; o.words_per_row = mask_bits_out ? (dim + 31) / 32 : wpr; bits_written = true; }
             } else {
                 o.rows = redirect ? redirect->rows : out_rows;
diff --git a/cuda_gcn_amd/host/module.h b/cuda_gcn_amd/host/module.h
--- a/cuda_gcn_amd/host/module.h
+++ b/cuda_gcn_amd/host/module.h
@@ -89,6 +89,8 @@
     int wpr = 0;
     bool out_grad_complete = false;
     uint32_t *mask_bits_out = nullptr;
+    uint32_t *keep_words = nullptr;
+    int64_t keep_words_bits = 0;
     const uint32_t *const *bwd_row_bits = nullptr;
     const gcnhip_graph *bwd_graph = nullptr;
     gcnhip_rowset *const *fwd_out_rows = nullptr;
@@ -114,6 +116,10 @@
     ~HipGraphSum() override;
     void forward(bool) override;
     void backward() override;
+    static size_t keep_words_needed(uint64_t elem_offset, size_t rows, int dim, int64_t *n_bits);
+private:
+    void draw_keep_words(gcnhip_gs_opts *o);
+public:
 private:
     uint16_t *bf_table = nullptr;
     int ld_bf = 0;
diff --git a/cuda_gcn_amd/host/options.cpp b/cuda_gcn_amd/host/options.cpp
--- a/cuda_gcn_amd/host/options.cpp
+++ b/cuda_gcn_amd/host/options.cpp
@@ -22,6 +22,7 @@
         o.exchange = !strcmp(e, "halo") ? 2 : (!strcmp(e, "allgather") ? 1 : (!strcmp(e, "auto") ? 0 : o.exchange));
     if (getenv("HIPGCN_NO_STRUCTURE_GROUPS")) o.structure_groups = false;
     if (getenv("HIPGCN_NO_MASK_BITS")) o.mask_bits = false;
+    if (getenv("HIPGCN_NO_HIDDEN_KEEP_WORDS")) o.hidden_keep_words = false;
     if (getenv("HIPGCN_NO_LOSS_EPILOGUE")) o.loss_epilogue = false;
     if (getenv("HIPGCN_NO_EVAL_FUSION")) o.eval_fusion = false;
     if (getenv("HIPGCN_NO_SLICE_TUNING")) o.slice_tuning = false;
diff --git a/cuda_gcn_amd/ops.py b/cuda_gcn_amd/ops.py
--- a/cuda_gcn_amd/ops.py
+++ b/cuda_gcn_amd/ops.py
@@ -10,7 +10,8 @@
 class GsOpts(C.Structure):
     _fields_ = [("rows", C.c_void_p), ("in_row_bits", C.c_void_p), ("accumulate", C.c_int), ("relu_dropout", C.c_int), ("training", C.c_int),
                 ("p", C.c_float), ("seed", C.c_uint64), ("d_epoch", C.c_void_p), ("elem_offset", C.c_uint64), ("keep_mask", C.c_void_p),
-                ("pos_bits", C.c_void_p), ("words_per_row", C.c_int), ("scaling", C.c_int), ("loss", C.c_void_p)]
+                ("pos_bits", C.c_void_p), ("words_per_row", C.c_int), ("scaling", C.c_int), ("loss", C.c_void_p),
+                ("keep_words", C.c_void_p), ("keep_bit0", C.c_uint64)]
 
 
 class GsLoss(C.Structure):
@@ -451,6 +452,34 @@
                                                                   elem_offset, km.ptr if km else None, bits.ptr, wpr), "graphsum_relu_dropout_bits")
         return out.download()[:, :dim], bits.download()
 
+    def keep_words(self, n_bits, p, seed=0, epoch=0, bit0=0):
+        words = self.buf(np.full(((n_bits + 127) // 128) * 4 + 4, 0xDEADBEEF, np.uint32))
+        ep = self.buf(np.array([epoch], np.uint32))
+        _ck(self.lib, self.lib.gcnhip_keep_words(self.ctx, words.ptr, n_bits, p, seed, ep.ptr, bit0), "gcnhip_keep_words")
+        return words
+
+    def graphsum_ex_relu_dropout(self, g, x, p, seed=0, epoch=0, elem_offset=0, words=False, rows=None, scaling=0, fill=np.nan):
+        x = np.asarray(x, np.float32)
+        dim = x.shape[1]
+        wpr = (dim + 31) // 32
+        xin = self.buf(x)
+        out = self.buf(np.full((g.n_rows, dim), fill, np.float32))
+        bits = self.buf(np.full((g.n_rows, wpr), 0xDEADBEEF, np.uint32))
+        g.reserve(dim)
+        ep = self.buf(np.array([epoch], np.uint32))
+        o = GsOpts()
+        o.rows = rows
+        o.scaling = int(scaling)
+        o.relu_dropout, o.training, o.p, o.seed, o.d_epoch, o.elem_offset = 1, 1, p, seed, ep.ptr, elem_offset
+        if rows is None:
+            o.pos_bits, o.words_per_row = bits.ptr, wpr
+        if words:
+            bit0 = elem_offset // 128 * 128
+            kw = self.keep_words(elem_offset - bit0 + g.n_rows * dim + 32, p, seed, epoch, bit0)
+            o.keep_words, o.keep_bit0 = kw.ptr, bit0
+        _ck(self.lib, self.lib.gcnhip_graphsum_ex(self.ctx, g.h, C.byref(o), xin.ptr, dim, out.ptr, dim, dim), "gcnhip_graphsum_ex")
+        return out.download(), bits.download()
+
     def matmul_bwd_fused_bits(self, a, b, dc, scale, bits):
         a, b, dc = (np.asarray(t, np.float32) for t in (a, b, dc))
         m, n = a.shape
diff --git a/include/gcnhip_driver.h b/include/gcnhip_driver.h
--- a/include/gcnhip_driver.h
+++ b/include/gcnhip_driver.h
@@ -50,7 +50,10 @@
     int words_per_row;
     int scaling;
     const struct gcnhip_gs_loss *loss;
+    const uint32_t *keep_words;
+    uint64_t keep_bit0;
 } gcnhip_gs_opts;
+int gcnhip_keep_words(gcnhip_ctx *ctx, uint32_t *words, int64_t n_bits, float p, uint64_t seed, const uint32_t *d_epoch, uint64_t bit0);
 typedef struct gcnhip_gs_loss {
     const int32_t *truth;
     float *grad; int ld_grad;
```

Result: no change. 350.3, median of 6 (+0.6%).
